# pangenome/povu

Hardware: AMD Instinct MI355X
Metric: edges/sec decomposed (flubble+PVST) (higher is better)
Workload: dtype u32

## Files before the change

include/povu_hip.h:

```cpp
#ifndef POVU_HIP_H
#define POVU_HIP_H

#include <stddef.h>
#include <stdint.h>

#ifdef __cplusplus
extern "C" {
#endif

#define POVU_HIP_NIL 0xFFFFFFFFu
#define POVU_SIDE_L 0
#define POVU_SIDE_R 1
#define POVU_TIP_NONE 0
#define POVU_TIP_L 1
#define POVU_TIP_R 2

typedef struct povu_hip_ctx povu_hip_ctx;
typedef struct povu_hip_forest povu_hip_forest;

int povu_hip_device_count(void);

povu_hip_ctx *povu_hip_create(int device, char *err, size_t errlen);
void povu_hip_destroy(povu_hip_ctx *ctx);
int povu_hip_release_workspace(povu_hip_ctx *ctx);
// ... 320 lines not shown
char *povu_hip_pvst_format(uint32_t n_pvst, const uint32_t *a_id, const uint32_t *z_id, const uint8_t *a_or,
			   const uint8_t *z_or, const uint32_t *parent, size_t *len);
char *povu_hip_pvst_format_fam(uint32_t n_pvst, const uint32_t *a_id, const uint32_t *z_id, const uint8_t *a_or,
			       const uint8_t *z_or, const uint32_t *parent, const uint8_t *fam, size_t *len);
void povu_hip_buffer_free(void *p);

typedef struct {
	uint32_t n;
	char *type;
	uint32_t *file_id;
	uint32_t *a_id, *z_id;
	uint8_t *a_or, *z_or;
	uint8_t *route;
	uint32_t *parent;
	uint32_t *height;
} povu_pvst_doc;
povu_pvst_doc *povu_pvst_parse(const char *text, size_t len, char *err, size_t errlen);

int povu_hip_gfa_write(const char *path, uint32_t n_vtx, const uint32_t *vid, uint32_t n_links, const uint32_t *v1,
		       const uint8_t *s1, const uint32_t *v2, const uint8_t *s2, char *err, size_t errlen);
void povu_pvst_doc_free(povu_pvst_doc *doc);

typedef struct {
	povu_hip_call_refs refs;
	uint32_t n_paths;
	const uint32_t *slot_of_path;
	const char *const *sample;
	const int64_t *slot_hap;
} povu_hip_call_names;
povu_hip_call_names *povu_hip_call_names_make(uint32_t n_paths, const char *const *path_name, uint32_t n_prefixes,
					      const char *const *prefix, char *err, size_t errlen);
void povu_hip_call_names_free(povu_hip_call_names *n);
int povu_hip_sites_add_tree(povu_hip_sites *s, uint32_t tree, uint32_t n, const uint32_t *id1, const uint32_t *id2,
			    const uint8_t *or1, const uint8_t *or2, const uint32_t *parent, const uint8_t *family);
povu_hip_sites *povu_hip_sites_of_docs(const povu_pvst_doc *const *docs, uint32_t n);
povu_hip_sites *povu_hip_forest_sites(const povu_hip_forest *f);
void povu_hip_sites_free(povu_hip_sites *s);
char *povu_hip_calls_vcf(const povu_hip_calls *c, const povu_hip_sites *sites, const povu_hip_call_names *names,
			 const char *const *path_name, const char *date, const char *only_prefix, uint32_t threads, size_t *len);
char *povu_hip_calls_vcf_profile(const povu_hip_calls *c, const povu_hip_sites *sites, const povu_hip_call_names *names,
				 const char *const *path_name, const char *date, const char *only_prefix, uint32_t threads, uint32_t profile,
				 size_t *len);
char *povu_hip_calls_vcf_rest(const povu_hip_calls *c, const povu_hip_sites *sites, const povu_hip_call_names *names,
			      const char *const *path_name, const char *date, const char *const *prefix, uint32_t n_prefixes, uint32_t threads,
			      uint32_t profile, size_t *len);

#define POVU_HIP_V_FOUND_FWD 0u
#define POVU_HIP_V_FOUND_REV 1u
#define POVU_HIP_V_ABSENT 2u
#define POVU_HIP_V_NO_AT 3u
#define POVU_HIP_V_BAD_STEP 4u
#define POVU_HIP_V_NO_SLOT 5u
#define POVU_HIP_V_MISSPELLED 6u
#define POVU_HIP_V_N_STATUS 6u
#define POVU_HIP_V_SPELL_NONE 0u
#define POVU_HIP_V_SPELL_WHOLE 1u
#define POVU_HIP_V_SPELL_ANCHORED 2u
#define POVU_HIP_V_SPELL_MISSPELLED 3u
#define POVU_HIP_V_FORWARD_ONLY 1u
#define POVU_HIP_V_SPELLING 2u
#define POVU_HIP_V_FORCE_TIER2 4u
typedef struct {
	uint64_t n_samples, n_records, n_alleles, n_steps, n_text_bytes, n_tasks, n_id_bytes;
	const char *const *sample;
	const uint64_t *rec_line;
	const uint64_t *rec_pos;
	const uint64_t *rec_id_off;
	const char *ids;
	const uint64_t *allele_off;
	const uint64_t *task_off;
	const uint64_t *step_off;
	const uint64_t *text_off;
	const uint8_t *allele_walk;
	const uint32_t *step_id;
	const uint8_t *step_or;
	const char *text;
	const uint32_t *task_record, *task_allele, *task_col, *task_phase;
} povu_hip_vcf_doc;
povu_hip_vcf_doc *povu_hip_vcf_parse(const char *text, size_t len, uint32_t threads, char *err, size_t errlen);
void povu_hip_vcf_doc_free(povu_hip_vcf_doc *d);
povu_hip_call_names *povu_hip_vcf_names_make(uint32_t n_paths, const char *const *path_name, char *err, size_t errlen);
int povu_hip_vcf_columns(const povu_hip_vcf_doc *doc, const povu_hip_call_names *names, uint32_t *col_first, uint32_t *col_slots);
typedef struct {
	uint32_t flags;
} povu_hip_vcf_opts;
typedef struct {
	uint64_t n_records, n_tasks, n_alleles;
	const uint8_t *task_status;
	const uint8_t *allele_spell;
	const uint8_t *rec_invalid;
	const uint8_t *rec_reason;
	const uint32_t *rec_allele, *rec_task;
	uint64_t n_status[POVU_HIP_V_N_STATUS];
	uint64_t n_invalid, n_misspelled;
	uint64_t n_tier2;
	double device_ms;
} povu_hip_vcf_report;
povu_hip_vcf_report *povu_hip_vcf_check(povu_hip_ctx *ctx, const povu_hip_vcf_doc *doc, const povu_hip_call_names *names,
					const povu_hip_vcf_opts *opts, char *err, size_t errlen);
void povu_hip_vcf_report_free(povu_hip_vcf_report *r);
char *povu_hip_vcf_report_text(const povu_hip_vcf_report *r, const povu_hip_vcf_doc *doc, const povu_hip_call_names *names,
			       size_t *report_len, char **summary, size_t *summary_len);

typedef struct {
	char name[48];
	double ms;
	uint32_t launches;
} povu_hip_stage_time;
int povu_hip_last_stage_times(const povu_hip_ctx *ctx, povu_hip_stage_time *out, int max);
uint32_t povu_hip_last_seq_redo(const povu_hip_ctx *ctx);
int povu_hip_last_black_only_classes(const povu_hip_ctx *ctx);
int povu_hip_last_narrow_counts(const povu_hip_ctx *ctx);
uint64_t povu_hip_wide_repeats(const povu_hip_ctx *ctx);
int povu_hip_last_laminar_check_ran(const povu_hip_ctx *ctx);
int povu_hip_last_crossings(povu_hip_ctx *ctx, uint32_t out[2]);
uint64_t povu_hip_last_links_processed(const povu_hip_ctx *ctx);

int povu_hip_debug_components(povu_hip_ctx *ctx, uint32_t *comp_of, uint32_t *local_idx);
int povu_hip_debug_tree(povu_hip_ctx *ctx, uint32_t comp, uint32_t *n_tree, uint32_t *gid, uint8_t *typ,
			uint32_t *par, uint32_t *cls);
int povu_hip_debug_edge_ids(povu_hip_ctx *ctx, uint32_t comp, uint32_t *n_tree, uint32_t *tree_edge_id);
int povu_hip_debug_walk_words(povu_hip_ctx *ctx, uint32_t out[3]);
int povu_hip_debug_stack(povu_hip_ctx *ctx, uint32_t comp, uint32_t *n, uint32_t *tree_vtx, uint32_t *cls,
			 uint32_t *next_seen);

#define POVU_HIP_SCAN_SUM 0
#define POVU_HIP_SCAN_MAX 1
#define POVU_HIP_SCAN_U64 2
#define POVU_HIP_SCAN_U8 3
#define POVU_HIP_SCAN_DIFF 4
#define POVU_HIP_SCAN_XOR_PAIR 5
#define POVU_HIP_SCAN_XOR_U128 6
#define POVU_HIP_SCAN_DIFF_U8 7
#define POVU_HIP_SCAN_MIXED_PAIR 8
#define POVU_HIP_SCAN_DIFF_U8_U8 9
#define POVU_HIP_SCAN_IN_PLACE 0x100
#define POVU_HIP_SCAN_N_DEV 0x200
int povu_hip_debug_scan(povu_hip_ctx *ctx, int op, const uint32_t *in, uint32_t *out, size_t n, const uint32_t *in2,
			uint32_t *out2, size_t n2);
int povu_hip_debug_sort(povu_hip_ctx *ctx, const uint32_t *keys, const uint32_t *vals, size_t n, unsigned bits,
			uint32_t *keys_out, uint32_t *vals_out);
int povu_hip_debug_compact(povu_hip_ctx *ctx, const uint8_t *flags, size_t n, uint32_t *out, uint32_t *count);
int povu_hip_debug_totals(povu_hip_ctx *ctx, const uint32_t *a, const uint32_t *b, size_t n, uint64_t tot[2]);
#define POVU_HIP_SEG_MIN 0
#define POVU_HIP_SEG_FIRST_LESS 1
#define POVU_HIP_SEG_LAST_LESS 2
int povu_hip_debug_segtree(povu_hip_ctx *ctx, const uint32_t *val, size_t n, const uint32_t *queries, size_t nq, uint32_t *out,
			   uint32_t *tree, uint32_t *P);
int povu_hip_debug_bitrank(povu_hip_ctx *ctx, const uint8_t *flags, size_t n, const uint32_t *pos, size_t nq, uint32_t *rank,
			   uint32_t *test, uint32_t *records);
int povu_hip_debug_append(povu_hip_ctx *ctx, const uint8_t *flags, size_t n, uint32_t *list, uint32_t *count);
int povu_hip_debug_list_rank(povu_hip_ctx *ctx, uint32_t n, const uint32_t *next, const uint8_t *w, const uint32_t *heads,
			     uint32_t nh, int mode, uint32_t bits, uint32_t *ra, uint32_t *rb);
double povu_hip_debug_scan_time(povu_hip_ctx *ctx, size_t n, int reps, int op);

uint64_t povu_hip_workspace_estimate(uint32_t n_vtx, uint32_t n_links, uint32_t n_components);
int povu_hip_workspace_breakdown(uint32_t n_vtx, uint32_t n_links, uint32_t n_components, uint64_t out[7]);
int povu_hip_prewarm(povu_hip_ctx *ctx, uint32_t n_vtx, uint32_t n_links, char *err, size_t errlen);
uint64_t povu_hip_leaf_workspace_estimate(uint32_t n_vtx, uint32_t n_components);

const char *povu_hip_version(void);

#ifdef __cplusplus
}
#endif
#endif
```

povu_amd/csrc/hip/context.hpp:

```cpp
#pragma once
#include "../../../include/povu_hip.h"

#include "forest_wire.hpp"
#include "graph_kernels.hpp"
#include "leaf_kernels.hpp"
#include "par_kernels.hpp"
#include "seq_kernels.hpp"
#include "sub_kernels.hpp"
#include "tree_kernels.hpp"

#include <map>
#include <memory>
#include <mutex>
#include <numeric>
#include <string>

using namespace povu_hip;

struct PinnedPool {
	struct Block {
		void *p;
		size_t cap;
		int seg;
	};
// ... 53 lines not shown
			return;
		if (from && from->shared_tag.empty()) {
			pool = from;
			p = static_cast<T *>(pool->get(m * sizeof(T), cap_bytes, &seg));
		} else {
			p = static_cast<T *>(malloc(m * sizeof(T)));
			if (!p)
				throw std::bad_alloc();
		}
		n = m;
	}
	void assign(size_t m, T v)
	{
		resize(m);
		std::fill(p, p + m, v);
	}
	void assign(const T *a, const T *b)
	{
		resize((size_t)(b - a));
		if (n)
			memcpy(p, a, n * sizeof(T));
	}
	T *data() { return p; }
	const T *data() const { return p; }
	T *begin() { return p; }
	const T *begin() const { return p; }
	size_t size() const { return n; }
	bool empty() const { return n == 0; }
	T &operator[](size_t i) { return p[i]; }
	const T &operator[](size_t i) const { return p[i]; }
};

struct povu_hip_forest {
	uint32_t total_components = 0;
	hipEvent_t ev0 = nullptr, ev1 = nullptr;
	bool pending = false;
	double pass_ms = -1.0;
	std::vector<hipEvent_t> more_events;
	std::once_flag ready_once;
	void wait_arrays()
	{
		if (pending) {
			if (ev1)
				(void)hipEventSynchronize(ev1);
			for (hipEvent_t e : more_events)
				(void)hipEventSynchronize(e);
			pending = false;
		}
	}
	void ready()
	{
		std::call_once(ready_once, [this] {
			wait_arrays();
			float ms = 0;
			if (ev0 && ev1 && pass_ms < 0 && hipEventElapsedTime(&ms, ev0, ev1) == hipSuccess)
				pass_ms = ms;
		});
	}
	std::shared_ptr<PinnedPool> pool;
	size_t meta_reserve = 0;
	static size_t meta_bytes(size_t n_trees) { return 64 + 32 * n_trees; }
	using Arrays = forest_wire::PvstArrays;
	static size_t block_bytes_for(size_t total) { return Arrays::layout(nullptr, total) + 64; }
	struct Block : Arrays {
		void *p = nullptr;
		size_t cap = 0, bytes = 0, total = 0;
		int seg = -1;
		std::shared_ptr<PinnedPool> pool;
		PinnedVec<uint32_t> sub_ai, sub_zi;
		PinnedVec<uint8_t> sub_fam;
		std::shared_ptr<SubForest> subx;
	};
	std::vector<Block> blocks;
	bool labels = false;
	Block &alloc(size_t total, void *q = nullptr, size_t cap = 0)
	{
		Block b;
		b.total = total, b.p = q, b.cap = cap;
		if (!q) {
			b.pool = pool;
			b.p = pool->get(block_bytes_for(total) + meta_bytes(meta_reserve), b.cap, &b.seg);
		}
		b.bytes = Arrays::layout(b.p, total, &b);
		blocks.push_back(std::move(b));
		return blocks.back();
	}
	void release_blocks()
	{
		for (auto &b : blocks)
			if (b.p && b.pool)
				b.pool->put(b.p, b.cap, b.seg);
		blocks.clear();
	}
	~povu_hip_forest()
	{
		std::call_once(ready_once, [this] { wait_arrays(); });
		if (ev0)
			(void)hipEventDestroy(ev0);
		if (ev1)
			(void)hipEventDestroy(ev1);
		for (hipEvent_t e : more_events)
			(void)hipEventDestroy(e);
		release_blocks();
		if (xblk && pool)
			pool->put(xblk, xblk_cap, xblk_seg);
	}
	struct Tree : forest_wire::TreeRecord {
		int blk = 0;
	};
	std::vector<Tree> trees;
	std::vector<uint64_t> hairpins;
	void *xblk = nullptr;
	size_t xblk_cap = 0;
	int xblk_seg = -1;
	const void *walk_ctx = nullptr;
	uint64_t walk_gen = 0;
};

struct PassPlan {
	uint32_t rank = 0, world = 1;
	bool hairpins = false, all_seq = false, seq_tree = false, par_tree = true, leaf_sub = false, all_sub = false;
	bool sorted_adj = false, force_redo = false, redo_odd = false;
	bool big_class_dfs = false, sparse_splitters = false, all_vertex_classes = false, check_laminar = false;
	bool timed = true, overlap_tail = false, heaviest_first = false;
};

struct LastPass {
	bool valid = false;
	PassPlan plan;
	uint32_t C = 0, seq_redo = 0;
	bool mixed = false, redo_pvst_only = false, stack_export_pending = false;
	bool narrow_counts = false;
	int narrow_forms = 0;
};

struct povu_hip_ctx {
	int device = 0;
	hipStream_t stream = nullptr;
	SideStream side;
	ResidentGraph g;
	SubArenas ws_sub;
	Arena ws, ws_b, ws2, ws_seq, ws_leaf, ws_walk, upload_tmp;
	HostScratch host;
	std::shared_ptr<PinnedPool> pool = std::make_shared<PinnedPool>();
	StageTimer timer;
	std::vector<povu_hip_stage_time> last_times;
	uint64_t last_links = 0;
	uint64_t wide_repeats = 0;
	CompState cs{};
	SeqWs sw{};
	ParWs pw{};
	TreeWs tw{};
	LastPass last;
	std::vector<uint32_t> shard_comp_ids;
	uint32_t shard_total_components = 0;
	Arena shard_buf;
	Arena graph_arena;
	hipEvent_t tail_done = nullptr;
	SideStream walk_side;
	bool tail_pending = false;
	void wait_tail()
	{
		if (tail_pending) {
			(void)hipEventSynchronize(tail_done);
			tail_pending = false;
		}
	}
	void quiesce()
	{
		if (tail_pending) {
			(void)hipStreamSynchronize(stream);
			wait_tail();
		}
	}
	Arena wk_ws, wk_out;
	Arena paths_buf;
	uint32_t *path_steps = nullptr;
	uint64_t *path_off = nullptr;
	uint32_t n_paths = 0;
	uint64_t n_path_steps = 0, paths_gen = 0;
	bool paths_valid = false;
	Arena tr_ws, tr_task, tr_trav, tr_steps;
	Arena seq_buf, cl_ws, cl_slot, cl_rec, cl_spell, cl_bytes;
	Arena iv_ws, iv_heads, iv_rows;
	Arena nm_ws;
	Arena pr_ws, pr_slab, pr_rows;
	Arena mg_ws, mg_rows;
	Arena ns_idx, ns_cls, ns_ws, ns_rec;
	Arena or_ws, or_view, or_inv, or_host, or_rows;
	Arena vc_ws, vc_hit;
	uint64_t *seq_off = nullptr;
	char *seq = nullptr;
	uint64_t seq_gen = 0;
	bool seq_valid = false;
	Arena part_arena;
	uint64_t xfer_h2d = 0, xfer_d2h = 0, xfer_peer_out = 0, xfer_peer_in = 0;
	struct Mapped {
		void *p;
		size_t bytes;
	};
	std::map<std::string, Mapped> attached;
};

struct XferScope {
	povu_hip_ctx *ctx;
	XferTally at;
	explicit XferScope(povu_hip_ctx *c) : ctx(c), at(xfer_tally()) {}
	~XferScope()
	{
		if (!ctx)
			return;
		const XferTally now = xfer_tally();
		ctx->xfer_h2d += now.h2d - at.h2d;
		ctx->xfer_d2h += now.d2h - at.d2h;
	}
};


void adopt_forest(povu_hip_forest &out, povu_hip_forest &m);

static inline void lpt_assign(const uint64_t *weights, uint32_t n, uint32_t world, uint32_t *order, uint32_t *owner)
{
	std::iota(order, order + n, 0u);
	std::stable_sort(order, order + n, [&](uint32_t a, uint32_t b) { return weights[a] > weights[b]; });
	std::vector<uint64_t> load(world, 0);
	for (uint32_t k = 0; k < n; k++) {
		const uint32_t c = order[k];
		uint32_t best = 0;
		for (uint32_t r = 1; r < world; r++)
			if (load[r] < load[best])
				best = r;
		owner[c] = best;
		load[best] += weights[c] + 1;
	}
}

void alloc_resident_graph(Arena &arena, ResidentGraph &g, uint32_t n_vtx, uint32_t n_links, bool tips_given);
void free_resident_graph(ResidentGraph &g);
void check_graph_size(uint32_t n_vtx, uint32_t n_links);
void set_err(char *err, size_t errlen, const std::string &msg);

struct Sizes {
	size_t V, E, Cmax, T, B, nS, slots;
	void set_components(size_t C) { Cmax = C, T = 2 * V + C, B = E + V + 2 * T; }
};
struct RowBNeeds {
	bool identity;
	bool sort_free;
	bool self_loops;
};
size_t rowb_carve_label(Arena *ar, const Sizes &z, CompState &cs);
size_t rowb_carve_reindex(Arena *ar, const Sizes &z, size_t C, const RowBNeeds &need, CompState &cs);
size_t carve_workspace(Arena *ar, int part, const Sizes &z, CompState &cs, SeqWs &sw, bool hairpins);
```

povu_amd/csrc/hip/debug_hooks.hip:

```cpp
#include "context.hpp"
#include "segtree.hpp"

#include <algorithm>
#include <numeric>

using namespace povu_hip;

namespace
{
constexpr size_t DBG_GUARD = 256;
constexpr int DBG_GUARD_BYTE = 0xC5, DBG_POISON_BYTE = 0xA7;
constexpr int DBG_RC_GUARD = 5;
struct DbgOut {
	size_t bytes = 0;
	int fill = DBG_GUARD_BYTE;
	bool on = true;
	char *base = nullptr;
	size_t span = 0;
	template <class T>
	T *data() const { return reinterpret_cast<T *>(base + DBG_GUARD); }
	void declare(Spans &take, hipStream_t s)
	{
		if (!on)
			return;
// ... 246 lines not shown
	for (uint32_t j = 0; j < 4 && t0 + j < n; j++)
		f |= (flags[t0 + j] ? 1u : 0u) << j;
	const uint32_t w0 = (BIDX * blockDim.x + (threadIdx.x & ~63u)) / 16u;
	bitrank_store_wave(rec + w0, f, w0 + (threadIdx.x & 63u) <= n / 64u);
}
__global__ void __launch_bounds__(256) k_dbg_bitrank_query(uint32_t n, const uint4 *__restrict__ rec, uint32_t nq, const uint32_t *__restrict__ x,
							   uint32_t *__restrict__ rank, uint32_t *__restrict__ test)
{
	for (uint32_t i = blockIdx.x * blockDim.x + threadIdx.x; i < nq; i += gridDim.x * blockDim.x) {
		const uint32_t p = x[i];
		rank[i] = bitrank(rec, p);
		if (p < n)
			test[i] = bitrank_test(rec, p) ? 1u : 0u;
	}
}
__global__ void __launch_bounds__(LIST_TPB) k_dbg_append(uint32_t n, const uint8_t *__restrict__ flags, uint32_t *__restrict__ list,
							  uint32_t *__restrict__ n_list)
{
	const uint32_t B0 = BIDX * LIST_SPAN;
	unsigned long long fw = 0;
#pragma unroll
	for (uint32_t it = 0; it < LIST_ITER; it++) {
		const uint32_t p0 = B0 + it * (LIST_TPB * 4u) + threadIdx.x * 4u;
		uint32_t f = 0;
		for (uint32_t j = 0; j < 4 && p0 + j < n; j++)
			f |= (flags[p0 + j] ? 1u : 0u) << j;
		fw |= (unsigned long long)f << (4 * it);
	}
	append_in_order(fw, B0, list, n_list);
}
constexpr size_t DBG_LOOKUP_MAX_N = (size_t(1) << 32) - (size_t(1) << 16);
unsigned dbg_query_blocks(size_t nq) { return (unsigned)std::min<size_t>(std::max<size_t>((nq + 255) / 256, 1), 4096); }
}

extern "C" int povu_hip_debug_segtree(povu_hip_ctx *ctx, const uint32_t *val, size_t n, const uint32_t *queries, size_t nq, uint32_t *out,
				      uint32_t *tree, uint32_t *P)
{
	if (!ctx || n > DBG_LOOKUP_MAX_N || nq >= (size_t(1) << 32) || (n && !val) || (nq && (!queries || !out)))
		return 1;
	for (size_t i = 0; i < nq; i++)
		if (queries[4 * i] > DBG_SEG_LAST || queries[4 * i + 2] > n)
			return 1;
	try {
		HIP_CHECK(hipSetDevice(ctx->device));
		hipStream_t s = ctx->stream;
		const size_t padded = (n + SEG_BLK - 1) / SEG_BLK * SEG_BLK, tw = SegTree::tree_words(n);
		Arena ar;
		DbgOut ot{tw * 4, DBG_POISON_BYTE}, oq{nq * 4};
		DbgScratch vals{(padded + SEG_BLK) * 4};
		DbgIn<uint32_t> dq{queries, 4 * nq};
		dbg_carve(ar, s, ot, oq, vals, dq);
		uint32_t *dv = static_cast<uint32_t *>(vals.p);
		if (n)
			HIP_CHECK(copy_async(dv, val, n * 4, hipMemcpyHostToDevice, s));
		if (padded > n)
			HIP_CHECK(hipMemsetAsync(dv + n, 0, (padded - n) * 4, s));
		SegTree st;
		st.tree = ot.data<uint32_t>();
		seg_build(st, dv, n, s);
		if (nq)
			KLAUNCH(k_dbg_seg_query, dim3(dbg_query_blocks(nq)), dim3(256), 0, s, st, (uint32_t)nq, reinterpret_cast<const uint4 *>(dq.dev), oq.data<uint32_t>());
		std::vector<uint32_t> ht(tw);
		HIP_CHECK(copy_async(ht.data(), ot.data<char>(), tw * 4, hipMemcpyDeviceToHost, s));
		if (nq)
			HIP_CHECK(copy_async(out, oq.data<char>(), nq * 4, hipMemcpyDeviceToHost, s));
		HIP_CHECK(hipStreamSynchronize(s));
		if (P)
			*P = st.P;
		if (tree)
			std::copy(ht.begin(), ht.begin() + 2 * (size_t)st.P, tree);
		if (!dbg_guards_intact(ot, s) || !dbg_guards_intact(oq, s))
			return DBG_RC_GUARD;
		const unsigned char *hb = reinterpret_cast<const unsigned char *>(ht.data());
		for (size_t i = 2 * (size_t)st.P * 4; i < tw * 4; i++)
			if (hb[i] != (unsigned char)DBG_POISON_BYTE)
				return DBG_RC_GUARD;
		return 0;
	} catch (const std::exception &) {
		return 2;
	}
}

extern "C" int povu_hip_debug_bitrank(povu_hip_ctx *ctx, const uint8_t *flags, size_t n, const uint32_t *pos, size_t nq, uint32_t *rank,
				      uint32_t *test, uint32_t *records)
{
	if (!ctx || n > DBG_LOOKUP_MAX_N || nq >= (size_t(1) << 32) || (n && !flags) || (nq && (!pos || !rank || !test)))
		return 1;
	for (size_t i = 0; i < nq; i++)
		if (pos[i] > n)
			return 1;
	try {
		HIP_CHECK(hipSetDevice(ctx->device));
		hipStream_t s = ctx->stream;
		const size_t n_rec = n / 64 + 1, tb = scan_tmp_bytes(n_rec + 1);
		Arena ar;
		DbgOut orec{(n_rec + 1) * 16, DBG_POISON_BYTE}, ocnt{(n_rec + 1) * 4, DBG_POISON_BYTE}, ork{nq * 4}, ots{nq * 4};
		DbgScratch tmp{tb};
		DbgIn<uint8_t> df{flags, n};
		DbgIn<uint32_t> dp{pos, nq};
		dbg_carve(ar, s, orec, ocnt, ork, ots, tmp, df, dp);
		uint4 *rec = orec.data<uint4>();
		const size_t waves = n / 256 + 1;
		KLAUNCH(k_dbg_bitrank_flags, dim3((unsigned)((waves * 64 + 255) / 256)), dim3(256), 0, s, (uint32_t)n, df.dev, rec);
		bitrank_build(rec, n_rec, ocnt.data<uint32_t>(), tmp.p, tb, s);
		if (nq) {
			KLAUNCH(k_dbg_bitrank_query, dim3(dbg_query_blocks(nq)), dim3(256), 0, s, (uint32_t)n, rec, (uint32_t)nq, dp.dev, ork.data<uint32_t>(),
				ots.data<uint32_t>());
			HIP_CHECK(copy_async(rank, ork.data<char>(), nq * 4, hipMemcpyDeviceToHost, s));
			HIP_CHECK(copy_async(test, ots.data<char>(), nq * 4, hipMemcpyDeviceToHost, s));
		}
		if (records)
			HIP_CHECK(copy_async(records, orec.data<char>(), (n_rec + 1) * 16, hipMemcpyDeviceToHost, s));
		HIP_CHECK(hipStreamSynchronize(s));
		return dbg_guards_intact(orec, s) && dbg_guards_intact(ocnt, s) && dbg_guards_intact(ork, s) && dbg_guards_intact(ots, s) ? 0 : DBG_RC_GUARD;
	} catch (const std::exception &) {
		return 2;
	}
}

extern "C" int povu_hip_debug_append(povu_hip_ctx *ctx, const uint8_t *flags, size_t n, uint32_t *list, uint32_t *count)
{
	if (!ctx || !count || n > DBG_LOOKUP_MAX_N || (n && (!flags || !list)))
		return 1;
	try {
		HIP_CHECK(hipSetDevice(ctx->device));
		hipStream_t s = ctx->stream;
		Arena ar;
		DbgOut ol{n * 4}, oc{4};
		DbgIn<uint8_t> df{flags, n};
		dbg_carve(ar, s, ol, oc, df);
		HIP_CHECK(hipMemsetAsync(oc.data<char>(), 0, 4, s));
		if (n)
			KLAUNCH(k_dbg_append, dim3((unsigned)((n + LIST_SPAN - 1) / LIST_SPAN)), dim3(LIST_TPB), 0, s, (uint32_t)n, df.dev, ol.data<uint32_t>(),
				oc.data<uint32_t>());
		if (n)
			HIP_CHECK(copy_async(list, ol.data<char>(), n * 4, hipMemcpyDeviceToHost, s));
		HIP_CHECK(copy_async(count, oc.data<char>(), 4, hipMemcpyDeviceToHost, s));
		HIP_CHECK(hipStreamSynchronize(s));
		if (!dbg_guards_intact(ol, s) || !dbg_guards_intact(oc, s))
			return DBG_RC_GUARD;
		return dbg_all_guard(list, std::min<size_t>(*count, n) * 4, n * 4) ? 0 : DBG_RC_GUARD;
	} catch (const std::exception &) {
		return 2;
	}
}

extern "C" int povu_hip_debug_list_rank(povu_hip_ctx *ctx, uint32_t n, const uint32_t *next, const uint8_t *w, const uint32_t *heads,
					uint32_t nh, int mode, uint32_t bits, uint32_t *ra, uint32_t *rb)
{
	if (!ctx || !next || !w || (nh && !heads) || !ra || (mode != 0 && !rb) || mode < 0 || mode > 1)
		return 1;
	try {
		HIP_CHECK(hipSetDevice(ctx->device));
		debug_list_rank(n, next, w, heads, nh, mode, bits, ra, rb, ctx->stream);
		return 0;
	} catch (const std::exception &) {
		return 2;
	}
}

extern "C" double povu_hip_debug_scan_time(povu_hip_ctx *ctx, size_t n, int reps, int op)
{
	if (!ctx || !n || reps <= 0)
		return -1.0;
	try {
		HIP_CHECK(hipSetDevice(ctx->device));
		hipStream_t s = ctx->stream;
		Arena ar;
		const size_t tb = scan_tmp_bytes(n);
		uint32_t *di = nullptr, *dout = nullptr;
		void *tmp = nullptr;
		carve(ar, [&](Spans &take) {
			take(n + 16, di, dout);
			take(tb, tmp);
		});
		HIP_CHECK(hipMemsetAsync(di, 1, n * 4, s));
		hipEvent_t e0, e1;
		HIP_CHECK(hipEventCreate(&e0));
		HIP_CHECK(hipEventCreate(&e1));
		for (int w = 0; w < 2; w++)
			op ? scan_exclusive_max_u32(di, dout, n, tmp, tb, s) : scan_exclusive_u32(di, dout, n, tmp, tb, s);
		HIP_CHECK(hipEventRecord(e0, s));
		for (int r = 0; r < reps; r++)
			op ? scan_exclusive_max_u32(di, dout, n, tmp, tb, s) : scan_exclusive_u32(di, dout, n, tmp, tb, s);
		HIP_CHECK(hipEventRecord(e1, s));
		HIP_CHECK(hipEventSynchronize(e1));
		float ms = 0;
		HIP_CHECK(hipEventElapsedTime(&ms, e0, e1));
		(void)hipEventDestroy(e0);
		(void)hipEventDestroy(e1);
		return (double)ms / reps;
	} catch (const std::exception &) {
		return -2.0;
	}
}

extern "C" int povu_hip_debug_components(povu_hip_ctx *ctx, uint32_t *comp_of, uint32_t *local_idx)
{
	if (!ctx || !ctx->last.valid)
		return 1;
	ctx->quiesce();
	try {
		HIP_CHECK(hipSetDevice(ctx->device));
		const uint32_t V = ctx->g.V, C = ctx->last.C;
		std::vector<uint32_t> pos(V), voff(C + 1);
		HIP_CHECK(hipMemcpy(comp_of, ctx->cs.comp_of, (size_t)V * 4, hipMemcpyDeviceToHost));
		if (ctx->cs.lean_identity)
			std::iota(pos.begin(), pos.end(), 0u);
		else
			HIP_CHECK(hipMemcpy(pos.data(), ctx->cs.pos, (size_t)V * 4, hipMemcpyDeviceToHost));
		HIP_CHECK(hipMemcpy(voff.data(), ctx->cs.voff, (size_t)(C + 1) * 4, hipMemcpyDeviceToHost));
		for (uint32_t v = 0; v < V; v++)
			local_idx[v] = pos[v] - voff[comp_of[v]];
		return 0;
	} catch (const std::exception &) {
		return 2;
	}
}

extern "C" int povu_hip_debug_tree(povu_hip_ctx *ctx, uint32_t comp, uint32_t *n_tree, uint32_t *gid, uint8_t *typ,
				   uint32_t *par, uint32_t *cls)
{
	if (!ctx || !ctx->last.valid || comp >= ctx->last.C || !n_tree)
		return 1;
	if (cls && ctx->last.mixed)
		return 4;
	ctx->quiesce();
	try {
		HIP_CHECK(hipSetDevice(ctx->device));
		uint32_t voff = 0, N = 0;
		HIP_CHECK(hipMemcpy(&voff, ctx->cs.voff + comp, 4, hipMemcpyDeviceToHost));
		HIP_CHECK(hipMemcpy(&N, ctx->sw.c_ntree + comp, 4, hipMemcpyDeviceToHost));
		*n_tree = N;
		const size_t tb = 2 * (size_t)voff + comp;
		if (gid)
			HIP_CHECK(hipMemcpy(gid, ctx->sw.t_gid + tb, (size_t)N * 4, hipMemcpyDeviceToHost));
		if (par)
			HIP_CHECK(hipMemcpy(par, ctx->sw.t_par + tb, (size_t)N * 4, hipMemcpyDeviceToHost));
		const bool par_cls = !ctx->last.plan.all_seq && (ctx->last.seq_redo == 0 || ctx->last.redo_pvst_only);
		if (cls && par_cls) {
			classes_to_tree_space(ctx->pw, ctx->stream);
			HIP_CHECK(hipStreamSynchronize(ctx->stream));
		}
		if (cls)
			HIP_CHECK(hipMemcpy(cls, (par_cls ? ctx->pw.gcls : ctx->sw.t_cls) + tb, (size_t)N * 4, hipMemcpyDeviceToHost));
		if (typ)
			HIP_CHECK(hipMemcpy(typ, ctx->sw.t_flags + tb, N, hipMemcpyDeviceToHost));
		return 0;
	} catch (const std::exception &) {
		return 2;
	}
}

extern "C" int povu_hip_debug_edge_ids(povu_hip_ctx *ctx, uint32_t comp, uint32_t *n_tree, uint32_t *tree_edge_id)
{
	if (!ctx || !ctx->last.valid || comp >= ctx->last.C || !n_tree)
		return 1;
	if (!ctx->last.plan.par_tree)
		return 3;
	if (ctx->last.mixed)
		return 4;
	uint32_t *dw = nullptr;
	ctx->quiesce();
	try {
		HIP_CHECK(hipSetDevice(ctx->device));
		uint32_t voff = 0, N = 0;
		HIP_CHECK(hipMemcpy(&voff, ctx->cs.voff + comp, 4, hipMemcpyDeviceToHost));
		HIP_CHECK(hipMemcpy(&N, ctx->sw.c_ntree + comp, 4, hipMemcpyDeviceToHost));
		*n_tree = N;
		if (!tree_edge_id || N == 0)
			return 0;
		const size_t T = 2 * (size_t)ctx->sw.V + ctx->last.C, tb = 2 * (size_t)voff + comp;
		HIP_CHECK(hipMalloc(reinterpret_cast<void **>(&dw), 2 * T * 4));
		HIP_CHECK(hipMemsetAsync(dw, 0, 2 * T * 4, ctx->stream));
		edge_id_weights(ctx->cs, ctx->sw, ctx->tw, dw, dw + T, ctx->stream);
		std::vector<uint32_t> w(N), tail(N), size(N);
		HIP_CHECK(copy_async(w.data(), dw + tb, (size_t)N * 4, hipMemcpyDeviceToHost, ctx->stream));
		HIP_CHECK(copy_async(tail.data(), dw + T + tb, (size_t)N * 4, hipMemcpyDeviceToHost, ctx->stream));
		HIP_CHECK(copy_async(size.data(), ctx->sw.t_size + tb, (size_t)N * 4, hipMemcpyDeviceToHost, ctx->stream));
		HIP_CHECK(hipStreamSynchronize(ctx->stream));
		HIP_CHECK(hipFree(dw));
		dw = nullptr;
		std::vector<uint32_t> closed((size_t)N + 1, 0);
		for (uint32_t t = 0; t < N; t++)
			closed[std::min<size_t>((size_t)t + size[t], N)] += tail[t];
		uint32_t before = 0;
		tree_edge_id[0] = POVU_NIL;
		for (uint32_t t = 0; t < N; t++) {
			before += w[t] + closed[t];
			if (t > 0)
				tree_edge_id[t] = t - 1 + before;
		}
		return 0;
	} catch (const std::exception &) {
		if (dw)
			(void)hipFree(dw);
		return 2;
	}
}

extern "C" int povu_hip_debug_walk_words(povu_hip_ctx *ctx, uint32_t out[3])
{
	if (!ctx || !ctx->last.valid || !out)
		return 1;
	if (!ctx->last.plan.par_tree)
		return 3;
	if (ctx->last.mixed)
		return 4;
	ctx->quiesce();
	try {
		HIP_CHECK(hipSetDevice(ctx->device));
// ... 40 lines not shown
```

povu_amd/csrc/hip/tree_kernels.hip:

```cpp
#include "tree_kernels.hpp"

#include <cstdlib>

#include <algorithm>
#include <type_traits>
#include <vector>

namespace povu_hip
{

#ifndef NIL
#define NIL POVU_NIL
#endif

static unsigned rank_bucket_bits(size_t n)
{
	if (const char *ev = getenv("POVU_HIP_RANK_BITS"))
		return (unsigned)std::min(6, std::max(2, atoi(ev)));
	(void)n;
	return 3u;
}
static constexpr uint32_t PK_END = 0x1FFFFFFFu, PK_STOP = 0x80000000u;
static constexpr uint32_t P0_END = 0x3FFFFFFFu, P0_W = 0x40000000u, P0_HEAD = 0x80000000u;
static constexpr uint32_t FT_NONE = 0x7FFFFFFFu, FT_HASH = 0x80000000u;
// ... 96 lines not shown
				h = hx(h, link_hash(le));
				continue;
			}
			if (first == NIL)
				first = at;
			const uint32_t w = ws[q], sb = o01[q].x;
			const uint32_t wl = (w & 1u) ? o01[q].y : sb, wh = (w & 1u) ? se[q] : o01[q].y;
			uint32_t nxt;
			if (se[q] - sb <= 8) {
				const uint32_t n = se[q] - sb, tl = wl - sb, th = wh - sb;
				uint4 c = make_uint4(0u, 0u, 0u, 0u);
				if (n > 4)
					c = load4_unaligned(lle + sb + 4);
				const uint32_t r[8] = {a[q].x, a[q].y, a[q].z, a[q].w, c.x, c.y, c.z, c.w};
				uint32_t tk = 0, first_tree = NIL, after = NIL;
#pragma unroll
				for (uint32_t k = 0; k < 8; k++)
					if (k >= tl && k < th && (r[k] & LLE_ID) == le)
						tk = k;
#pragma unroll
				for (uint32_t k = 0; k < 8; k++)
					if (k < n && (r[k] & LLE_TREE)) {
						if (first_tree == NIL)
							first_tree = k;
						if (k > tk && after == NIL)
							after = k;
					}
				nxt = sb + (after != NIL ? after : (first_tree < tk ? first_tree : tk));
			} else {
				const uint32_t t = wl + find_link_slot(loff, lle, w, le) - 1;
				nxt = t;
				for (uint32_t jj = t + 1; jj < se[q] && nxt == t; jj++)
					if (lle[jj] & LLE_TREE)
						nxt = jj;
				for (uint32_t jj = sb; jj < t && nxt == t; jj++)
					if (lle[jj] & LLE_TREE)
						nxt = jj;
			}
			pk[at] = rank_pack(nxt, 1u, b);
		}
	}
	const bool nz = !hzero(h);
	if (nz)
		hside[S] = h;
	ft[S] = (first == NIL ? FT_NONE : first) | (nz ? FT_HASH : 0u);
}
__device__ __forceinline__ uint32_t comp_root_side(const unsigned long long *start_key, const uint32_t *voff, uint32_t c)
{
	unsigned long long k = start_key[c];
	return k == ~0ull ? 2 * voff[c] : (uint32_t)(k & 0xFFFFFFFFu);
}
__global__ void k_tour_ends(uint32_t C, const uint32_t *__restrict__ voff, const unsigned long long *__restrict__ start_key,
			    const uint32_t *__restrict__ loff, const uint32_t *__restrict__ ladj, const uint32_t *__restrict__ lle,
			    uint32_t *__restrict__ pk, uint32_t *__restrict__ heads)
{
	uint32_t c = BIDX * blockDim.x + threadIdx.x;
	if (c >= C)
		return;
	const uint32_t r = comp_root_side(start_key, voff, c), sb = loff[r & ~1u], se = loff[(r & ~1u) + 2], mid = loff[r];
	uint32_t a_first = NIL, a_last = NIL;
	for (uint32_t j = mid; j < se; j++)
		if (lle[j] & LLE_TREE) {
			if (a_first == NIL)
				a_first = j;
			a_last = j;
		}
	for (uint32_t j = sb; j < mid; j++)
		if (lle[j] & LLE_TREE) {
			if (a_first == NIL)
				a_first = j;
			a_last = j;
		}
	heads[c] = a_first;
	if (a_first == NIL)
		return;
	pk[arc_twin(loff, ladj, lle, a_last)] = P0_END;
	atomicOr(&pk[a_first], P0_HEAD);
}
template <int HOPS>
__global__ void k_wyllie(uint32_t n, const uint32_t *__restrict__ nxt_in, const uint32_t *__restrict__ a_in,
			 const uint32_t *__restrict__ b_in, uint32_t *__restrict__ nxt_out, uint32_t *__restrict__ a_out,
			 uint32_t *__restrict__ b_out, const uint32_t *__restrict__ n_dev)
{
	uint32_t i = BIDX * blockDim.x + threadIdx.x;
	if (i >= n || (n_dev && i >= *n_dev))
		return;
	uint32_t nx = nxt_in[i], a = a_in[i], b = b_in ? b_in[i] : 0;
#pragma unroll
	for (int hop = 0; hop < HOPS; hop++) {
		if (nx == NIL)
			break;
		a += a_in[nx];
		if (b_in)
			b += b_in[nx];
		nx = nxt_in[nx];
	}
	nxt_out[i] = nx;
	a_out[i] = a;
	if (b_out)
		b_out[i] = b;
}
static int list_rank(uint32_t n, unsigned bits, uint32_t *nxtA, uint32_t *nxtB, uint32_t *aA, uint32_t *aB, uint32_t *bA,
		     uint32_t *bB, hipStream_t s, const uint32_t *n_dev = nullptr)
{
	int cur = 0;
	const bool small = n < (1u << 21);
	const unsigned launches = small ? (bits + 2) / 3 : (bits + 1) / 2;
	for (unsigned r = 0; r < launches; r++) {
		uint32_t *ni = cur ? nxtB : nxtA, *no = cur ? nxtA : nxtB, *ai = cur ? aB : aA, *ao = cur ? aA : aB;
		uint32_t *bi = cur ? bB : bA, *bo = cur ? bA : bB;
		if (small)
			LAUNCH(k_wyllie<7>, n, s, n, ni, ai, bi, no, ao, bo, n_dev);
		else
			LAUNCH(k_wyllie<3>, n, s, n, ni, ai, bi, no, ao, bo, n_dev);
		cur ^= 1;
	}
	return cur;
}

static constexpr uint32_t RANK_TOP = 8192;
struct RankLevelArgs {
	uint32_t n;
	uint32_t m;
	uint32_t hbase;
	uint32_t M;
};
template <bool L0>
__device__ __forceinline__ uint32_t rank_lane_start(uint32_t id, const RankLevelArgs &A, unsigned b, const uint32_t *__restrict__ pk0,
						    const uint32_t *__restrict__ heads)
{
	if (id < A.m) {
		const uint32_t x = bucket_splitter(id, b);
		if (x >= A.n)
			return NIL;
		if (L0)
			return (pk0[x] & P0_HEAD) ? NIL : x;
		return x >= A.hbase ? NIL : x;
	}
	return L0 ? heads[id - A.m] : A.hbase + (id - A.m);
}
template <bool EVT3>
__device__ __forceinline__ void rank_l0_weights(uint32_t x, uint32_t p, uint32_t &wa, uint32_t &wb)
{
	if (EVT3) {
		const uint32_t t = x % 3u;
		wa = t == 0 ? 2u : 0u;
		wb = t == 0 ? 2u : ((t == 1 && (p & P0_W)) ? 0u - 2u : 0u - 1u);
	} else {
		wa = (p & P0_W) ? 1u : 0u;
		wb = wa ? 1u : 0xFFFFFFFFu;
	}
}
static constexpr uint32_t REC_MAX = 0xFFFFu;
template <bool L0, bool TWO, bool EVT3 = false>
__global__ void k_rank_up(RankLevelArgs A, unsigned b, const uint32_t *__restrict__ nx_in, const uint32_t *__restrict__ a_in,
			  const uint32_t *__restrict__ b_in, const uint32_t *__restrict__ heads, uint32_t *__restrict__ nx_out,
			  uint32_t *__restrict__ a_out, uint32_t *__restrict__ b_out, uint2 *__restrict__ rec, uint32_t *__restrict__ ovf)
{
	const uint32_t id = BIDX * blockDim.x + threadIdx.x;
	if (id >= A.M)
		return;
	uint32_t x = rank_lane_start<L0>(id, A, b, nx_in, heads);
	uint32_t sa = 0, sb = 0, out = PK_END | PK_STOP;
	bool big = false;
	if (x != NIL) {
		uint32_t p;
		bool stop;
		do {
			p = nx_in[x];
			if (L0) {
				uint32_t wa, wb;
				rank_l0_weights<EVT3>(x, p, wa, wb);
				if (TWO) {
					big |= sa > REC_MAX || sa - sb > REC_MAX;
					rec[x] = make_uint2(id, sa | ((sa - sb) << 16));
				} else {
					rec[x] = make_uint2(id, sa);
				}
				sa += wa;
				if (TWO)
					sb += wb;
				x = p & P0_END;
				stop = rank_l0_stop(x, b);
			} else {
				sa += a_in[x];
				if (TWO)
					sb += b_in[x];
				x = p & PK_END;
				stop = (p & PK_STOP) != 0;
			}
		} while (!stop);
		if (x != (L0 ? P0_END : PK_END)) {
			const uint32_t q = x >> b;
			out = q | (is_splitter(q, b) ? PK_STOP : 0u);
		}
	}
	nx_out[id] = out;
	a_out[id] = sa;
	if (TWO)
		b_out[id] = sb;
	if (L0 && TWO && big)
		*ovf = 1u;
}
template <bool EVT3>
__global__ void k_rank_l0_fallback(RankLevelArgs A, unsigned b, const uint32_t *__restrict__ pk, const uint32_t *__restrict__ heads,
				   const uint32_t *__restrict__ ra, const uint32_t *__restrict__ rb, uint2 *__restrict__ rec,
				   const uint32_t *__restrict__ ovf)
{
	if (!*ovf)
		return;
	for (uint32_t id = BIDX * blockDim.x + threadIdx.x; id < A.M; id += gridDim.x * blockDim.x) {
		uint32_t x = rank_lane_start<true>(id, A, b, pk, heads);
		if (x == NIL)
			continue;
		uint32_t sa = ra[id], sb = rb[id];
		do {
			const uint32_t p = pk[x];
			uint32_t wa, wb;
			rank_l0_weights<EVT3>(x, p, wa, wb);
			rec[x] = make_uint2(sa, sb);
			sa -= wa;
			sb -= wb;
			x = p & P0_END;
		} while (!rank_l0_stop(x, b));
	}
}
template <bool TWO>
__global__ void k_rank_down(RankLevelArgs A, unsigned b, const uint32_t *__restrict__ nx_in, uint32_t *a_io, uint32_t *b_io,
			    const uint32_t *__restrict__ ra, const uint32_t *__restrict__ rb)
{
	const uint32_t id = BIDX * blockDim.x + threadIdx.x;
	if (id >= A.M)
		return;
	uint32_t x = rank_lane_start<false>(id, A, b, nx_in, nullptr);
	if (x == NIL)
		return;
	uint32_t sa = ra[id], sb = TWO ? rb[id] : 0, p;
	do {
		p = nx_in[x];
		const uint32_t wa = a_io[x];
		a_io[x] = sa;
		sa -= wa;
		if (TWO) {
			const uint32_t wb = b_io[x];
			b_io[x] = sb;
			sb -= wb;
		}
		x = p & PK_END;
	} while (!(p & PK_STOP));
}
template <bool TWO>
__global__ void __launch_bounds__(1024) k_rank_top(uint32_t n, const uint32_t *__restrict__ nx_in, uint32_t *a_io, uint32_t *b_io)
{
	__shared__ uint32_t nx[RANK_TOP], sa[RANK_TOP], sb[TWO ? RANK_TOP : 1];
	for (uint32_t i = threadIdx.x; i < n; i += blockDim.x) {
		const uint32_t p = nx_in[i] & PK_END;
		nx[i] = p == PK_END ? NIL : p;
		sa[i] = a_io[i];
		if (TWO)
			sb[i] = b_io[i];
	}
	__syncthreads();
	constexpr int PER = RANK_TOP / 1024;
	for (uint32_t span = 1; span < n; span <<= 1) {
		uint32_t tn[PER], ta[PER], tb[PER];
#pragma unroll
		for (int k = 0; k < PER; k++) {
			const uint32_t i = threadIdx.x + k * 1024;
			tn[k] = NIL, ta[k] = 0, tb[k] = 0;
			if (i < n && nx[i] != NIL) {
				const uint32_t j = nx[i];
				tn[k] = nx[j];
				ta[k] = sa[j];
				if (TWO)
					tb[k] = sb[j];
			}
		}
		__syncthreads();
#pragma unroll
		for (int k = 0; k < PER; k++) {
			const uint32_t i = threadIdx.x + k * 1024;
			if (i < n && nx[i] != NIL) {
				nx[i] = tn[k];
				sa[i] += ta[k];
				if (TWO)
					sb[i] += tb[k];
			}
		}
		__syncthreads();
	}
	for (uint32_t i = threadIdx.x; i < n; i += blockDim.x) {
		a_io[i] = sa[i];
		if (TWO)
			b_io[i] = sb[i];
	}
}
__global__ void k_rank_unpack_next(uint32_t n, const uint32_t *__restrict__ nx_in, uint32_t *__restrict__ out)
{
	uint32_t i = BIDX * blockDim.x + threadIdx.x;
	if (i < n) {
		const uint32_t p = nx_in[i] & PK_END;
		out[i] = p == PK_END ? NIL : p;
	}
}

struct RankBufs {
	uint32_t *pk;
	uint32_t *heads;
	uint32_t *nx, *wa, *wb;
	uint32_t *tA, *tB, *tC;
};
static constexpr int RANK_MAX_LEVELS = 12;
static size_t rank_pool_words(size_t n, size_t nh) { return n / 2 + 4 * nh + 64; }

struct L0Ranks {
	const uint32_t *ra, *rb, *fin;
	uint32_t M;
};
__device__ __forceinline__ uint32_t l0_at(const L0Ranks &R, uint2 rec, bool want = true) { return want && rec.x < R.M ? rec.x : 0u; }
__device__ __forceinline__ uint32_t rank_l0(const L0Ranks &R, uint2 rec, uint32_t ra) { return (rec.x < R.M ? ra : 0u) - rec.y; }
__device__ __forceinline__ uint32_t rank_l0_a(const L0Ranks &R, uint2 rec, bool fin, uint32_t ra)
{
	return fin ? rec.x : (rec.x < R.M ? ra : 0u) - (rec.y & REC_MAX);
}
__device__ __forceinline__ uint2 rank_l0_pair(const L0Ranks &R, uint2 rec, bool fin, uint32_t ra, uint32_t rb)
{
	const bool in = rec.x < R.M;
	const uint32_t pa = rec.y & REC_MAX;
	return fin ? rec : make_uint2((in ? ra : 0u) - pa, (in ? rb : 0u) - pa + (rec.y >> 16));
}
__device__ __forceinline__ uint32_t rank_l0(const L0Ranks &R, uint2 rec) { return rank_l0(R, rec, R.ra[l0_at(R, rec)]); }
__device__ __forceinline__ uint2 rank_l0_pair(const L0Ranks &R, uint2 rec, bool fin)
{
	const uint32_t i = l0_at(R, rec, !fin);
	return rank_l0_pair(R, rec, fin, R.ra[i], R.rb[i]);
}

template <bool TWO, bool EVT3 = false>
static L0Ranks list_rank_splitters(uint32_t n, unsigned b, uint2 *rec, uint32_t *ovf, uint32_t nh, RankBufs &rb, hipStream_t s)
{
	if (n >= P0_END)
		throw HipError("list ranking: more than 2^30 elements (graph too large for the packed walk)");
	RankLevelArgs lv[RANK_MAX_LEVELS];
	uint32_t *nxp[RANK_MAX_LEVELS + 1], *wap[RANK_MAX_LEVELS + 1], *wbp[RANK_MAX_LEVELS + 1];
	int levels = 0;
	size_t used = 0;
	const size_t pool = rank_pool_words(n, nh);
	nxp[0] = rb.pk, wap[0] = wbp[0] = nullptr;
	uint32_t cur_n = n, hbase = 0;
	for (;;) {
		RankLevelArgs &A = lv[levels];
		A.n = cur_n;
		A.m = (cur_n + (1u << b) - 1) >> b;
		A.hbase = hbase;
		A.M = A.m + nh;
		if (used + A.M > pool)
			throw HipError("list ranking: level pool exhausted (internal sizing bug)");
		nxp[levels + 1] = rb.nx + used, wap[levels + 1] = rb.wa + used, wbp[levels + 1] = rb.wb + used;
		used += A.M;
		levels++;
		hbase = A.m;
		const uint32_t next_n = A.M;
		if (next_n <= RANK_TOP || next_n > cur_n / 2 || levels == RANK_MAX_LEVELS) {
			cur_n = next_n;
			break;
		}
		cur_n = next_n;
	}
	if (TWO)
		HIP_CHECK(hipMemsetAsync(ovf, 0, 4, s));
	for (int L = 0; L < levels; L++) {
		const RankLevelArgs &A = lv[L];
		if (L == 0)
			LAUNCH((k_rank_up<true, TWO, EVT3>), A.M, s, A, b, nxp[0], nullptr, nullptr, rb.heads, nxp[1], wap[1], wbp[1], rec, ovf);
		else
			LAUNCH((k_rank_up<false, TWO>), A.M, s, A, b, nxp[L], wap[L], wbp[L], nullptr, nxp[L + 1], wap[L + 1], wbp[L + 1],
			       nullptr, nullptr);
	}
	const uint32_t nt = cur_n;
	if (nt <= RANK_TOP) {
		KLAUNCH((k_rank_top<TWO>), dim3(1), dim3(1024), 0, s, nt, nxp[levels], wap[levels], wbp[levels]);
	} else {
		LAUNCH(k_rank_unpack_next, nt, s, nt, nxp[levels], rb.tA);
		HIP_CHECK(copy_async(rb.tB, wap[levels], (size_t)nt * 4, hipMemcpyDeviceToDevice, s));
		if (TWO)
			HIP_CHECK(copy_async(rb.tC, wbp[levels], (size_t)nt * 4, hipMemcpyDeviceToDevice, s));
		uint32_t *nA = rb.tA, *nB = nxp[levels], *aA = rb.tB, *aB = wap[levels], *bA = rb.tC, *bB = wbp[levels];
		const int side = list_rank(nt, bits_for(nt) + 1, nA, nB, aA, aB, TWO ? bA : nullptr, TWO ? bB : nullptr, s);
		if (side == 0) {
			HIP_CHECK(copy_async(wap[levels], aA, (size_t)nt * 4, hipMemcpyDeviceToDevice, s));
			if (TWO)
				HIP_CHECK(copy_async(wbp[levels], bA, (size_t)nt * 4, hipMemcpyDeviceToDevice, s));
		}
	}
	for (int L = levels - 1; L >= 1; L--) {
		const RankLevelArgs &A = lv[L];
		LAUNCH((k_rank_down<TWO>), A.M, s, A, b, nxp[L], wap[L], wbp[L], wap[L + 1], wbp[L + 1]);
	}
	if (TWO)
		KLAUNCH((k_rank_l0_fallback<EVT3>), dim3(std::min(nblk(lv[0].M), 2048u)), dim3(TPB), 0, s, lv[0], b, rb.pk, rb.heads, wap[1],
			wbp[1], rec, ovf);
	return L0Ranks{wap[1], TWO ? wbp[1] : nullptr, TWO ? ovf : nullptr, lv[0].M};
}

template <bool TWO>
__global__ void k_rank_resolve(uint32_t n, const uint2 *__restrict__ rec, L0Ranks R, uint32_t *__restrict__ ra, uint32_t *__restrict__ rb)
{
	const uint32_t x = BIDX * blockDim.x + threadIdx.x;
	if (x >= n)
		return;
	if (TWO) {
		const uint2 r = rank_l0_pair(R, rec[x], *R.fin != 0);
		ra[x] = r.x;
		rb[x] = r.y;
	} else {
		ra[x] = rank_l0(R, rec[x]);
	}
}
void debug_list_rank(uint32_t n, const uint32_t *next, const uint8_t *w, const uint32_t *heads, uint32_t nh, int mode,
		     unsigned bits, uint32_t *ra, uint32_t *rb, hipStream_t s)
{
	if (n == 0 || n >= P0_END)
		throw HipError("debug_list_rank: n must be in [1, 2^30)");
	const unsigned b = bits ? std::min(6u, std::max(2u, bits)) : rank_bucket_bits(n);
	std::vector<uint32_t> pk(n);
	for (uint32_t x = 0; x < n; x++) {
		if (next[x] != NIL && next[x] >= n)
			throw HipError("debug_list_rank: successor out of range");
		pk[x] = (next[x] == NIL ? P0_END : next[x]) | (w[x] ? P0_W : 0u);
	}
	for (uint32_t h = 0; h < nh; h++)
		if (heads[h] != NIL) {
			if (heads[h] >= n)
				throw HipError("debug_list_rank: head out of range");
			pk[heads[h]] |= P0_HEAD;
		}
	const size_t pool = rank_pool_words(n, nh);
	Arena ar;
	ar.reserve(Arena::padded(n + 16, 4) * 3 + Arena::padded(n + 16, 8) + Arena::padded(nh + 1, 4) + 6 * Arena::padded(pool, 4) + 8192, false);
	RankBufs rbf{};
	rbf.pk = ar.take<uint32_t>(n + 16);
	rbf.heads = ar.take<uint32_t>(nh + 1);
	for (uint32_t **q : {&rbf.nx, &rbf.wa, &rbf.wb, &rbf.tA, &rbf.tB, &rbf.tC})
		*q = ar.take<uint32_t>(pool);
	uint32_t *da = ar.take<uint32_t>(n + 16), *db = ar.take<uint32_t>(n + 16), *ovf = ar.take<uint32_t>(4);
	uint2 *rec = ar.take<uint2>(n + 16);
	HIP_CHECK(copy_async(rbf.pk, pk.data(), (size_t)n * 4, hipMemcpyHostToDevice, s));
	if (nh)
		HIP_CHECK(copy_async(rbf.heads, heads, (size_t)nh * 4, hipMemcpyHostToDevice, s));
	if (mode == 0) {
		const L0Ranks R = list_rank_splitters<false>(n, b, rec, nullptr, nh, rbf, s);
		LAUNCH(k_rank_resolve<false>, n, s, n, rec, R, da, nullptr);
	} else {
		const L0Ranks R = list_rank_splitters<true, true>(n, b, rec, ovf, nh, rbf, s);
		LAUNCH(k_rank_resolve<true>, n, s, n, rec, R, da, db);
	}
	HIP_CHECK(copy_async(ra, da, (size_t)n * 4, hipMemcpyDeviceToHost, s));
	if (mode != 0)
		HIP_CHECK(copy_async(rb, db, (size_t)n * 4, hipMemcpyDeviceToHost, s));
	HIP_CHECK(hipStreamSynchronize(s));
}

static constexpr uint32_t T0_RBIT = 0x80000000u;
static constexpr uint32_t BS_POS = 0x3FFFFFFFu, BS_NOARC = 0x80000000u, BS_HASH_L = 0x40000000u, BS_HASH_R = 0x80000000u;
__global__ void k_t0_parents(uint32_t V, const uint2 *__restrict__ trec, L0Ranks R, const uint32_t *__restrict__ ckey,
			     const uint32_t *__restrict__ voff, const uint32_t *__restrict__ loff, const uint32_t *__restrict__ ladj,
			     const uint32_t *__restrict__ lle,
			     const uint32_t *__restrict__ ft, const uint32_t *__restrict__ heads,
			     uint4 *__restrict__ t0seg, uint2 *__restrict__ fstr, uint4 *__restrict__ xrec, uint32_t C,
			     const unsigned long long *__restrict__ start_key, uint32_t *__restrict__ err, uint8_t *__restrict__ multi)
{
	uint32_t g = BIDX * blockDim.x + threadIdx.x;
	if (g < V)
		*reinterpret_cast<uint16_t *>(multi + 2 * g) = 0;
	if (g < C) {
		const uint32_t r = comp_root_side(start_key, voff, g), L = 2 * (voff[g + 1] - voff[g] - 1);
		t0seg[r >> 1] = make_uint4(NIL, (r & 1u) ? T0_RBIT : 0u, 0u, L ? L - 1 : 0u);
		const uint32_t h = heads[g];
		if (h == NIL ? L != 0 : rank_l0(R, trec[h]) != L - 1)
			atomicExch(err, 1u);
	}
	if (g >= V)
		return;
	const uint32_t sb = loff[2 * g], sm = loff[2 * g + 1], se = loff[2 * g + 2];
	const uint2 f2 = *reinterpret_cast<const uint2 *>(ft + 2 * g);
	uint32_t at_e = NIL, dmin = 0xFFFFFFFFu, dmax = 0u;
	uint32_t a_l = NIL, a_r = NIL, d_l = 0u, d_r = 0u;
	for (uint32_t at0 = sb; at0 < se; at0 += 4) {
		const uint32_t *r32 = reinterpret_cast<const uint32_t *>(trec + at0);
		const uint4 lw4 = load4_unaligned(lle + at0), r01 = load4_unaligned(r32), r23 = load4_unaligned(r32 + 4);
		const uint32_t lws[4] = {lw4.x, lw4.y, lw4.z, lw4.w};
		const uint2 rs[4] = {make_uint2(r01.x, r01.y), make_uint2(r01.z, r01.w), make_uint2(r23.x, r23.y), make_uint2(r23.z, r23.w)};
		bool tree[4];
		uint32_t ds[4];
#pragma unroll
		for (uint32_t q = 0; q < 4; q++) {
			tree[q] = at0 + q < se && (lws[q] & LLE_TREE);
			ds[q] = R.ra[l0_at(R, rs[q], tree[q])];
		}
		landed(ds[0], ds[1], ds[2], ds[3]);
#pragma unroll
		for (uint32_t q = 0; q < 4; q++)
			ds[q] = rank_l0(R, rs[q], ds[q]);
#pragma unroll
		for (uint32_t q = 0; q < 4; q++) {
			if (!tree[q])
				continue;
			if (ds[q] < dmin) {
				dmin = ds[q];
				at_e = at0 + q;
			}
			dmax = max(dmax, ds[q]);
			if (at0 + q < sm) {
				if (a_l == NIL)
					a_l = at0 + q, d_l = ds[q];
			} else if (a_r == NIL) {
				a_r = at0 + q, d_r = ds[q];
			}
		}
	}
	const uint32_t hbits = ((f2.x & FT_HASH) ? BS_HASH_L : 0u) | ((f2.y & FT_HASH) ? BS_HASH_R : 0u);
	if (at_e == NIL) {
		fstr[g] = make_uint2(BS_NOARC, hbits);
		return;
	}
	const uint32_t c = ckey[g], root = comp_root_side(start_key, voff, c);
	const uint32_t L = 2 * (voff[c + 1] - voff[c] - 1), abase = 2 * (voff[c] - c);
	if ((root >> 1) == g) {
		const bool far_r = !(root & 1u);
		const uint32_t a1 = far_r ? a_r : a_l, d1 = far_r ? d_r : d_l;
		fstr[g] = a1 == NIL ? make_uint2(BS_NOARC, hbits) : make_uint2((abase + (L - 1 - d1)) & BS_POS, ((abase + L) & BS_POS) | hbits);
		return;
	}
	const uint32_t p_in = abase + (L - 2 - dmax), p_out = abase + (L - 1 - dmin);
	t0seg[g] = make_uint4(ladj[at_e], (lle[at_e] & LLE_ID) | (at_e >= sm ? T0_RBIT : 0u), p_in, p_out);
	{
		const bool ent_r = at_e >= sm;
		const uint32_t a1 = ent_r ? a_l : a_r, d1 = ent_r ? d_l : d_r, a3 = ent_r ? a_r : a_l, d3 = ent_r ? d_r : d_l;
		const uint32_t end = a3 != at_e ? abase + (L - 1 - d3) : p_out;
		fstr[g] = a1 == NIL ? make_uint2(BS_NOARC, hbits) : make_uint2((abase + (L - 1 - d1)) & BS_POS, (end & BS_POS) | hbits);
	}
	if ((f2.x | f2.y) & FT_HASH)
		atomicOr(reinterpret_cast<unsigned long long *>(&xrec[p_in >> 6]), 1ull << (p_in & 63u));
}
__global__ void k_tour_values(uint32_t V, const uint4 *__restrict__ t0seg, const uint32_t *__restrict__ ft,
			      const ulonglong2 *__restrict__ hside, const uint4 *__restrict__ xrec, ulonglong2 *__restrict__ xval)
{
	uint32_t g = BIDX * blockDim.x + threadIdx.x;
	if (g >= V)
		return;
	const uint2 f2 = *reinterpret_cast<const uint2 *>(ft + 2 * g);
	if (!((f2.x | f2.y) & FT_HASH))
		return;
	const uint4 r = t0seg[g];
	if (r.x == NIL)
		return;
	const ulonglong2 z = make_ulonglong2(0ull, 0ull);
	xval[bitrank(xrec, r.z)] = hx((f2.x & FT_HASH) ? hside[2 * g] : z, (f2.y & FT_HASH) ? hside[2 * g + 1] : z);
}
static constexpr uint32_t PB_BRIDGE = 0x80000000u;
static constexpr uint32_t CLASS_BUDGET = 256;
static constexpr uint32_t CS_VISITED = 0x40000000u;
__global__ void k_bridges(uint32_t V, const uint4 *__restrict__ t0seg, const uint2 *__restrict__ fstr,
			  const ulonglong2 *__restrict__ xps, const uint4 *__restrict__ xrec,
			  const ulonglong2 *__restrict__ hside, const uint32_t *__restrict__ loff, const uint32_t *__restrict__ lle,
			  const uint32_t *__restrict__ ckey, const uint32_t *__restrict__ cproc,
			  uint8_t *multi, uint32_t *__restrict__ cstate, uint2 *__restrict__ dps)
{
	const uint32_t g = BIDX * blockDim.x + threadIdx.x;
	if (g >= V)
		return;
	auto stretch = [&](uint32_t p, uint32_t q) {
		const uint32_t rp = bitrank(xrec, p), rq = bitrank(xrec, q);
		return rp == rq ? make_ulonglong2(0ull, 0ull) : hx(xps[rp], xps[rq]);
	};
	const uint4 r = t0seg[g];
	const uint32_t Se = (2 * g) | (r.y >> 31), Sf = Se ^ 1u, c = ckey[g];
	const bool proc = cproc[c] != 0;
	uint32_t pvE;
	if (r.x == NIL) {
		pvE = NIL;
	} else if (hzero(stretch(r.z, r.w + 1))) {
		pvE = r.x | PB_BRIDGE;
	} else {
		pvE = r.x;
		multi[Se] = 1;
		multi[r.x] = 1;
	}
	const uint2 fs = fstr[g];
	ulonglong2 x = (fs.y & ((Sf & 1u) ? BS_HASH_R : BS_HASH_L)) ? hside[Sf] : make_ulonglong2(0ull, 0ull);
	if (!(fs.x & BS_NOARC))
		x = hx(x, stretch(fs.x & BS_POS, fs.y & BS_POS));
	uint32_t pvF;
	if (hzero(x)) {
		pvF = Se | PB_BRIDGE;
	} else {
		pvF = Se;
		multi[Sf] = 1;
		multi[Se] = 1;
	}
	const bool entryE = proc && (pvE & PB_BRIDGE), entryF = proc && (pvF & PB_BRIDGE);
	const uint32_t csE = proc ? (pvE | (entryE ? CS_VISITED : 0u)) : NIL, csF = proc ? (pvF | (entryF ? CS_VISITED : 0u)) : NIL;
	uint2 recE = make_uint2(NIL, 0u), recF = make_uint2(NIL, 0u);
	if (entryE && pvE != NIL) {
		const uint32_t p = pvE & ~PB_BRIDGE;
		recE.x = p;
		uint32_t le = r.y & ~T0_RBIT, lo = loff[p], hi = loff[p + 1];
		while (lo < hi) {
			const uint32_t mid = (lo + hi) >> 1;
			if ((lle[mid] & LLE_ID) < le)
				lo = mid + 1;
			else
				hi = mid;
		}
		recE.y = lo - loff[p] + 1;
	}
	if (entryF)
		recF.x = Se;
	const bool e_first = !(Se & 1u);
	*reinterpret_cast<uint2 *>(cstate + 2 * g) = e_first ? make_uint2(csE, csF) : make_uint2(csF, csE);
	*reinterpret_cast<uint4 *>(dps + 2 * g) = e_first ? make_uint4(recE.x, recE.y, recF.x, recF.y) : make_uint4(recF.x, recF.y, recE.x, recE.y);
}


static constexpr uint32_t EL_ITER = LIST_ITER, EL_SIDES = LIST_SPAN;
static_assert(TPB == (int)LIST_TPB, "append_in_order is written for workgroups of 256");
__global__ void __launch_bounds__(TPB) k_entry_list(uint32_t nS, const uint32_t *__restrict__ pbr ,
						     const uint8_t *__restrict__ multi, const uint32_t *__restrict__ ckey,
						     const uint32_t *__restrict__ cproc, uint32_t *__restrict__ entry_list,
						     uint32_t *__restrict__ n_entry)
{
	const uint32_t B0 = BIDX * EL_SIDES;
	unsigned long long fw = 0;
#pragma unroll
	for (uint32_t it = 0; it < EL_ITER; it++) {
		const uint32_t S0 = B0 + it * (TPB * 4u) + threadIdx.x * 4u;
		uint32_t f = 0;
		if (S0 + 4 <= nS) {
			const uint4 pb = *reinterpret_cast<const uint4 *>(pbr + S0);
			const uint32_t mu = *reinterpret_cast<const uint32_t *>(multi + S0);
			const uint2 ck = *reinterpret_cast<const uint2 *>(ckey + (S0 >> 1));
			const uint32_t c0 = cproc[ck.x] ? 1u : 0u, c1 = cproc[ck.y] ? 1u : 0u;
			f = (((mu & 0xFFu) && (pb.x & PB_BRIDGE)) ? c0 : 0u) | ((((mu & 0xFF00u) && (pb.y & PB_BRIDGE)) ? c0 : 0u) << 1) |
			    ((((mu & 0xFF0000u) && (pb.z & PB_BRIDGE)) ? c1 : 0u) << 2) | ((((mu & 0xFF000000u) && (pb.w & PB_BRIDGE)) ? c1 : 0u) << 3);
		} else {
			for (uint32_t S = S0; S < nS; S++)
				f |= ((multi[S] && (pbr[S] & PB_BRIDGE) && cproc[ckey[S >> 1]]) ? 1u : 0u) << (S - S0);
		}
		fw |= (unsigned long long)f << (4 * it);
	}
// ... 260 lines not shown
						base = NIL;
					}
					chunk_base[n_chunks] = base;
				}
				base = sgpr(base);
				if (base == NIL) {
					pool_ok = false;
					return;
				}
				n_chunks++;
			}
			__syncthreads();
			if (lane < 32)
				wstk[wstk_addr(ev + lane, chunk_base)] = ring[(ev + lane) & 63u];
			lds_lo = ev + 32;
		}
		if (lane == 0)
			ring[d & 63u] = make_uint2(side, jn);
		depth = d + 1;
	};
	auto set_parent = [&](uint32_t side, uint32_t par) {
		const uint32_t kk = side - win_lo;
		if (HOT && kk < W_WIN) {
			if (lane == 0)
				win_par[kk] = par | W_DIRTY;
			return true;
		}
		if (lane == 0)
			wpar[side] = par;
		return false;
	};
#define W_INLINE_CAND(rr, idx, out)                                                                                            \
	do {                                                                                                                    \
		uint32_t v__ = (rr).c0;                                                                                         \
		v__ = (idx) == 1 ? (rr).c1 : v__;                                                                               \
		v__ = (idx) == 2 ? (rr).c2 : v__;                                                                               \
		v__ = (idx) == 3 ? (rr).c3 : v__;                                                                               \
		v__ = (idx) == 4 ? (rr).c4 : v__;                                                                               \
		v__ = (idx) == 5 ? (rr).c5 : v__;                                                                               \
		(out) = (idx) < (rr).n ? v__ : NIL;                                                                             \
	} while (0)
	constexpr uint32_t W_TRIAL = 512;
	uint32_t n_gen = 0, n_hot = 0;
	if (HOT) {
		for (;;) {
			if (n_gen >= W_TRIAL && n_hot < n_gen)
				break;
			n_gen++;
#define W_HOT 1
#include "walk_step.inc"
#undef W_HOT
		}
	}
	for (;;) {
#define W_HOT 0
#include "walk_step.inc"
#undef W_HOT
	}
}
__global__ void k_walk_finish(uint32_t nS, const uint32_t *__restrict__ wpar, const uint32_t *__restrict__ pbr,
			      const uint32_t *__restrict__ loff, const uint32_t *__restrict__ ladj, uint2 *__restrict__ dps)
{
	uint32_t S = BIDX * blockDim.x + threadIdx.x;
	if (S >= nS)
		return;
	const uint32_t p = wpar[S];
	if (p == W_UNVIS || (pbr[S] & PB_BRIDGE))
		return;
	uint32_t slot = 0;
	if (S != (p ^ 1u)) {
		const uint32_t lo = loff[p], hi = loff[p + 1];
		for (uint32_t k = lo; k < hi; k++)
			if (ladj[k] == S) {
				slot = k - lo + 1;
				break;
			}
	}
	dps[S] = make_uint2(p, slot);
}

__device__ __forceinline__ uint32_t leave_event(uint32_t p, bool p_is_far) { return 3 * (p >> 1) + (p_is_far ? 1u : 2u); }
__global__ void k_events(uint32_t V, const uint2 *__restrict__ dps, const uint32_t *__restrict__ loff,
			 const uint32_t *__restrict__ ladj, const uint32_t *__restrict__ ckey, const uint32_t *__restrict__ cproc,
			 uint32_t *__restrict__ pk, uint32_t *__restrict__ heads, unsigned b, uint8_t *__restrict__ merged,
			 uint32_t *__restrict__ sdl)
{
	const uint32_t g = BIDX * blockDim.x + threadIdx.x;
	if (g >= V)
		return;
	sdl[g] = 0;
	if (g == 0)
		sdl[V] = sdl[V + 1] = 0;
	const uint32_t A = 3 * g;
	const uint4 d4 = *reinterpret_cast<const uint4 *>(dps + 2 * g);
	if (d4.x != 2 * g + 1 && d4.z != 2 * g) {
		pk[A] = pk[A + 1] = pk[A + 2] = P0_END;
		merged[g] = 1;
		return;
	}
	const uint32_t o = d4.x == 2 * g + 1 ? 2 * g : 2 * g + 1, e = o ^ 1u;
	const uint32_t p = (e & 1u) ? d4.z : d4.x, slot_e = (e & 1u) ? d4.w : d4.y;
	auto child_behind = [&](uint32_t par, uint32_t lo, uint32_t n, uint32_t from) {
		for (uint32_t k = from; k <= n; k += 4) {
			const uint4 x = load4_unaligned(ladj + lo + k - 1);
			const uint32_t rem = n + 1 - k;
			const uint2 r0 = dps[x.x];
			const uint2 r1 = rem > 1 ? dps[x.y] : make_uint2(NIL, 0u);
			const uint2 r2 = rem > 2 ? dps[x.z] : make_uint2(NIL, 0u);
			const uint2 r3 = rem > 3 ? dps[x.w] : make_uint2(NIL, 0u);
			if (r0.x == par && r0.y == k)
				return x.x;
			if (r1.x == par && r1.y == k + 1)
				return x.y;
			if (r2.x == par && r2.y == k + 2)
				return x.z;
			if (r3.x == par && r3.y == k + 3)
				return x.w;
		}
		return NIL;
	};
	const uint2 s01 = *reinterpret_cast<const uint2 *>(loff + 2 * g);
	const uint32_t s2 = loff[2 * g + 2];
	const uint32_t lo_o = (o & 1u) ? s01.y : s01.x, n_o = ((o & 1u) ? s2 : s01.y) - lo_o;
	const uint32_t lo_e = (e & 1u) ? s01.y : s01.x, n_e = ((e & 1u) ? s2 : s01.y) - lo_e;
	const uint32_t c_o = child_behind(o, lo_o, n_o, 1u);
	const uint32_t ns_o = child_behind(e, lo_e, n_e, 1u);
	uint32_t after_e = NIL;
	if (p != NIL) {
		const uint32_t lo_p = loff[p], n_p = loff[p + 1] - lo_p;
		const uint32_t ns_e = child_behind(p, lo_p, n_p, slot_e + 1);
		after_e = ns_e != NIL ? 3 * (ns_e >> 1) : leave_event(p, dps[p].x == (p ^ 1u));
	}
	uint32_t enter = rank_pack(c_o != NIL ? 3 * (c_o >> 1) : A + 1, 0u, b);
	if (p == NIL) {
		const uint32_t comp = ckey[g];
		if (cproc[comp]) {
			enter |= P0_HEAD;
			heads[comp] = A;
		}
	}
	pk[A] = enter;
	if (ns_o != NIL) {
		pk[A + 1] = rank_pack(3 * (ns_o >> 1), 0u, b);
		pk[A + 2] = rank_pack(after_e, 0u, b);
		merged[g] = 0;
	} else {
		pk[A + 1] = rank_pack(after_e, 1u, b);
		pk[A + 2] = P0_END;
		merged[g] = 1;
	}
}

template <typename OC, typename SC, typename IC>
__global__ void k_tree_emit(uint32_t nS, const uint2 *__restrict__ erec, L0Ranks R, const uint8_t *__restrict__ merged,
			    const uint2 *__restrict__ dps, const uint32_t *__restrict__ ckey,
			    const uint32_t *__restrict__ cproc, const uint32_t *__restrict__ voff,
			    const unsigned long long *__restrict__ start_key, const uint32_t *__restrict__ gid_s,
			    uint32_t *__restrict__ t_gid, uint8_t *__restrict__ t_flags, uint32_t *__restrict__ t_par,
			    uint32_t *__restrict__ t_size, uint32_t *__restrict__ t_depth, uint32_t *__restrict__ side_tidx,
			    uint32_t C, uint32_t *__restrict__ c_ntree, OC *__restrict__ ordcnt, uint32_t *__restrict__ hi0,
			    uint32_t *__restrict__ mpre, SC *__restrict__ srccnt, uint32_t *__restrict__ sdl,
			    IC *__restrict__ incnt)
{
	uint32_t S = BIDX * blockDim.x + threadIdx.x;
	if (S == 0) {
		const uint32_t T = 2 * (nS >> 1) + C;
		hi0[T] = NIL;
		srccnt[T] = srccnt[T + 1] = 0;
		incnt[T] = incnt[T + 1] = 0;
	}
	if (S < C) {
		const uint32_t Nr = 2 * (voff[S + 1] - voff[S]), tr = 2 * voff[S] + S;
		if (!cproc[S]) {
			c_ntree[S] = 0;
			t_size[tr + Nr] = 0;
			srccnt[tr + Nr] = 0;
			incnt[tr + Nr] = 0;
		} else {
			const uint32_t hr = start_key[S] != ~0ull ? 1u : 0u;
			c_ntree[S] = Nr + hr;
			if (hr) {
				t_gid[tr] = NIL;
				t_flags[tr] = 2 | TF_ROOT;
				t_par[tr] = NIL;
				t_size[tr] = Nr + 1;
				incnt[tr] = 0;
				if (t_depth)
					t_depth[tr] = 0;
				mpre[tr] = tr;
				ordcnt[tr] = 0;
				hi0[tr] = NIL;
			} else {
				t_size[tr + Nr] = 0;
				srccnt[tr + Nr] = 0;
				incnt[tr + Nr] = 0;
			}
		}
	}
	const uint32_t g = S;
	if (g >= (nS >> 1))
		return;
	const uint32_t c = ckey[g], v0 = voff[c];
	const uint32_t tb = 2 * v0 + c;
	if (!cproc[c]) {
		const uint32_t t = tb + 2 * (g - v0);
		store2_unaligned(t_size + t, 0u, 0u);
		zero2(srccnt + t);
		zero2(incnt + t);
		*reinterpret_cast<uint2 *>(side_tidx + 2 * g) = make_uint2(NIL, NIL);
		return;
	}
	const uint32_t Nh = 2 * (voff[c + 1] - v0), hd = start_key[c] != ~0ull ? 1u : 0u;
	const bool fin = *R.fin != 0;
	const uint4 r01 = load4_unaligned(reinterpret_cast<const uint32_t *>(erec + 3 * g));
	const uint2 r2 = erec[3 * g + 2];
	const bool two_leaves = !merged[g];
	const uint4 d4 = *reinterpret_cast<const uint4 *>(dps + 2 * g);
	const uint32_t o = d4.x == 2 * g + 1 ? 2 * g : 2 * g + 1, e = o ^ 1u;
	const uint32_t p = (e & 1u) ? d4.z : d4.x;
	const bool has_p = p != NIL;
	const uint32_t pp = has_p ? p : e;
	const uint2 r_p = erec[3 * (pp >> 1)], d_p = dps[pp];
	const uint2 r0 = make_uint2(r01.x, r01.y), r1 = make_uint2(r01.z, r01.w);
	const uint32_t i0 = l0_at(R, r0, !fin);
	uint32_t a0 = R.ra[i0], b0 = R.rb[i0], a1 = R.ra[l0_at(R, r1, !fin)], a2 = R.ra[l0_at(R, r2, !fin && two_leaves)], a_p = R.ra[l0_at(R, r_p, !fin && has_p)];
	landed(a0, b0, a1, a2, a_p);
	const uint2 ent = rank_l0_pair(R, r0, fin, a0, b0), lv_o = make_uint2(rank_l0_a(R, r1, fin, a1), 0u);
	const uint32_t lv_e2 = rank_l0_a(R, r2, fin, a2), ent_p = rank_l0_a(R, r_p, fin, a_p);
	const uint32_t pre_e = Nh - ent.x, depth_e = 0u - ent.y;
	const uint32_t lv_e = two_leaves ? lv_e2 : lv_o.x;
	const uint32_t size_o = ent.x - 1 - lv_o.x, size_e = ent.x - lv_e;
	uint32_t par_e;
	if (!has_p)
		par_e = hd ? 0u : NIL;
	else
		par_e = hd + (Nh - ent_p) + (d_p.x == (p ^ 1u) ? 1u : 0u);
	const uint32_t l = hd + pre_e, t = tb + l;
	const uint32_t gid = gid_s[g];
	store2_unaligned(t_gid + t, gid, gid);
	t_flags[t] = (uint8_t)((e & 1u) | (par_e == NIL ? TF_ROOT : 0u));
	t_flags[t + 1] = (uint8_t)((o & 1u) | TF_BLACK);
	store2_unaligned(t_par + t, par_e, l);
	store2_unaligned(t_size + t, size_e, size_o);
	zero2(incnt + t);
	if (t_depth)
		store2_unaligned(t_depth + t, depth_e + hd, depth_e + 1 + hd);
	store2_unaligned(mpre + t, tb + (depth_e + hd) + (Nh + hd) - l - size_e, tb + (depth_e + 1 + hd) + (Nh + hd) - (l + 1) - size_o);
	*reinterpret_cast<uint2 *>(side_tidx + 2 * g) = (e & 1u) ? make_uint2(t + 1, t) : make_uint2(t, t + 1);
	if (sdl) {
		const uint32_t gray = (size_e - 1 - size_o) / 2, black = (size_o + 1) / 2, gs = v0 + pre_e / 2;
		if (gray) {
			atomicAdd(&sdl[gs], gray);
			atomicAdd(&sdl[gs + black], 0u - gray - black);
			atomicAdd(&sdl[gs + size_e / 2], black);
		}
	}
}
#ifndef POVU_BE_ITER
#define POVU_BE_ITER 8
#endif
static constexpr uint32_t BE_ITER = POVU_BE_ITER, BE_SIDES = TPB * BE_ITER;
template <bool EMIT, typename IC>
__device__ __forceinline__ uint32_t side_back_edges(uint32_t S, uint32_t p, uint32_t at,
						    const uint32_t *__restrict__ loff, const uint32_t *__restrict__ ladj,
						    const uint2 *__restrict__ dps, const uint32_t *__restrict__ side_tidx,
						    const uint32_t *__restrict__ ckey, const uint32_t *__restrict__ voff,
						    const uint32_t *__restrict__ t_par, uint32_t *__restrict__ b_src,
						    uint32_t *__restrict__ b_tgt, uint32_t *__restrict__ b_ord,
						    const uint8_t *__restrict__ dupflag, IC *__restrict__ incnt, uint32_t &highest,
						    uint32_t *first2)
{
	uint32_t n = 0;
	const uint32_t c = ckey[S >> 1], root = 2 * voff[c] + c;
	const uint32_t lo = loff[S], hi = loff[S + 1];
	auto out = [&](uint32_t tgt) {
		if (EMIT) {
			b_src[at + n] = p;
			b_tgt[at + n] = tgt;
			b_ord[at + n] = n;
			if (sizeof(IC) == 4 || tgt != root)
				incnt_add(incnt, tgt);
		} else {
			highest = min(highest, tgt);
			if (n < 2)
				first2[n] = tgt;
		}
		n++;
	};
	if (lo == hi) {
		if (p == root || t_par[p] != 0)
			out(root);
		return n;
	}
	const uint32_t dp = dps[S].x;
	bool loop_seen = false;
	for (uint32_t k0 = lo; k0 < hi; k0 += 4) {
		const uint4 o4 = load4_unaligned(ladj + k0);
		const uint32_t rem = hi - k0;
		const uint32_t os[4] = {o4.x, o4.y, o4.z, o4.w};
		const uint32_t xs[4] = {side_tidx[o4.x], rem > 1 ? side_tidx[o4.y] : NIL, rem > 2 ? side_tidx[o4.z] : NIL,
					rem > 3 ? side_tidx[o4.w] : NIL};
#pragma unroll
		for (uint32_t q = 0; q < 4; q++) {
			if (q >= rem)
				break;
			const uint32_t k = k0 + q, o = os[q], x = xs[q];
			if (o == (S ^ 1)) {
				if (dp == o && !loop_seen)
					out(x);
				loop_seen = true;
				continue;
			}
			if (x > p || o == dp)
				continue;
			bool dup = false;
			if (dupflag) {
				dup = dupflag[k] != 0;
			} else {
				for (uint32_t j = lo; j < k; j++)
					if (ladj[j] == o) {
						dup = true;
						break;
					}
			}
			if (!dup)
				out(x);
		}
	}
	return n;
}
template <typename OC, typename IC>
__global__ void __launch_bounds__(TPB) k_back_edges(uint32_t nS, const uint32_t *__restrict__ loff, const uint32_t *__restrict__ ladj,
						     const uint2 *__restrict__ dps, const uint32_t *__restrict__ side_tidx,
						     const uint32_t *__restrict__ ckey, const uint32_t *__restrict__ voff,
						     const uint32_t *__restrict__ t_par, uint32_t *__restrict__ total_out,
						     uint32_t *__restrict__ b_src, uint32_t *__restrict__ b_tgt,
						     uint32_t *__restrict__ b_ord, const uint8_t *__restrict__ dupflag,
						     OC *__restrict__ ordcnt, uint32_t *__restrict__ hi0, IC *__restrict__ incnt,
						     uint32_t cap)
{
	const uint32_t S0 = BIDX * BE_SIDES + threadIdx.x;
	__shared__ uint32_t first2[BE_ITER][TPB][2];
	__shared__ uint8_t cnt8[BE_ITER][TPB];
	uint32_t n = 0;
	for (uint32_t it = 0; it < BE_ITER; it++) {
		const uint32_t S = S0 + it * TPB;
		const uint32_t p = S < nS ? side_tidx[S] : NIL;
		uint32_t k = 0;
		if (p != NIL) {
			uint32_t highest = NIL;
			k = side_back_edges<false, IC>(S, p, 0, loff, ladj, dps, side_tidx, ckey, voff, t_par, b_src, b_tgt, b_ord, dupflag, incnt, highest,
						   first2[it][threadIdx.x]);
			ordcnt[p] = (OC)k;
			hi0[p] = highest;
			n += k;
		}
		cnt8[it][threadIdx.x] = (uint8_t)min(k, 255u);
	}
	__shared__ uint32_t wsum[TPB / 64], base;
	uint32_t all;
	const uint32_t before = block_exclusive_scan<TPB / 64>(n, wsum, all, ScanOp<0>{});
	if (threadIdx.x == 0)
		base = all ? atomicAdd(total_out, all) : 0u;
	__syncthreads();
	if (!n || base + all > cap)
		return;
	uint32_t at = base + before;
	for (uint32_t it = 0; it < BE_ITER; it++) {
		const uint32_t k = cnt8[it][threadIdx.x];
		if (!k)
			continue;
		const uint32_t S = S0 + it * TPB, p = side_tidx[S];
		if (k <= 2) {
			uint32_t root = NIL;
			if constexpr (sizeof(IC) == 1) {
				const uint32_t c = ckey[S >> 1];
// ... 119 lines not shown
		if (groups & 1)
			spans(n, p...);
	};
	auto take = [&](size_t n, auto *&...p) {
		if (groups & 2)
			spans(n, p...);
	};
	const size_t nS = 2 * V + 2, NA = std::max<size_t>(4 * V, 2 * E) + 8;
	const size_t NSL = std::max<size_t>(2 * V + 2 * E, 4 * V) + 16;
	if (groups & 1)
		spans.bytes_for(tw.dvis_slots, std::max(2 * E, 2 * V) + 16);
	take1(nS, tw.side_tidx);
	take1(nS, tw.dps);
	take(2 * E + 16, tw.dist);
	take(NA / 64 + 4, tw.xrec);
	take(NA / 64 + 4, tw.xrank);
	if (groups & 2)
		spans.bytes_for(tw.evt, NA * 8);
	take(V + 2, tw.t0seg);
	take(nS, tw.entry_ps, tw.entry_list, tw.be_cnt);
	take(nS, tw.dvis);
	take(nS + 2 * E + 8, tw.wadj);
	take(Cmax + 2, tw.cproc);
	take(NSL, tw.rk_pk);
	take(Cmax + 2, tw.rk_heads);
	const size_t pool_b = Arena::padded(rank_pool_words(NSL, Cmax + 1), 4);
	const size_t xv_b = Arena::padded(std::max<size_t>(V + 2, E + 8) + 8, 16);
	const WalkBytes wb(nS);
	char *blk = nullptr;
	if (groups & 2)
		spans.bytes_for(blk, o.walk_inline ? std::max(6 * pool_b + 2 * xv_b, wb.total()) : 6 * pool_b + 2 * xv_b);
	if (groups & 2)
		tw.walk_inline = o.walk_inline;
	if (blk) {
		uint32_t **pools[6] = {&tw.rk_nx, &tw.rk_wa, &tw.rk_wb, &tw.rk_tA, &tw.rk_tB, &tw.rk_tC};
		for (int k = 0; k < 6; k++)
			*pools[k] = reinterpret_cast<uint32_t *>(blk + (size_t)k * pool_b);
		tw.xval = reinterpret_cast<decltype(tw.xval)>(blk + 6 * pool_b);
		tw.xps = reinterpret_cast<decltype(tw.xps)>(blk + 6 * pool_b + xv_b);
		if (o.walk_inline) {
			tw.wrec = reinterpret_cast<decltype(tw.wrec)>(blk);
			tw.wstk = reinterpret_cast<decltype(tw.wstk)>(blk + wb.rec);
			tw.wpar = reinterpret_cast<decltype(tw.wpar)>(blk + wb.rec + wb.stk);
		} else {
			tw.wrec = nullptr;
			tw.wstk = nullptr;
			tw.wpar = nullptr;
		}
	}
}

size_t tree_workspace_bytes(size_t V, size_t E, size_t Cmax, int groups, const StageWsOpts &o)
{
	TreeWs tmp{};
	return measure([&](Spans &take) { tree_spans(tmp, V, E, Cmax, groups, o, take); }) + (1 << 20);
}

void tree_carve(Arena &ar, TreeWs &tw, size_t V, size_t E, size_t Cmax, int groups, const StageWsOpts &o)
{
	Spans take{&ar};
	tree_spans(tw, V, E, Cmax, groups, o, take);
}

size_t walk_workspace_bytes(size_t V) { return WalkBytes(2 * V + 2).total() + 4096; }

size_t stage_workspace_bytes(size_t V, size_t E, size_t Cmax, const StageWsOpts &o)
{
	return par_workspace_bytes(V, E, Cmax, 1, o) + tree_workspace_bytes(V, E, Cmax, 1, o) +
	       std::max(tree_workspace_bytes(V, E, Cmax, 2, o), par_workspace_bytes(V, E, Cmax, 2, o));
}
void stage_workspace_carve(Arena &ar, ParWs &pw, TreeWs &tw, size_t V, size_t E, size_t Cmax, const StageWsOpts &o)
{
	par_carve(ar, pw, V, E, Cmax, 1, o);
	tree_carve(ar, tw, V, E, Cmax, 1, o);
	const size_t shared = ar.used();
	tree_carve(ar, tw, V, E, Cmax, 2, o);
	const size_t tree_end = ar.used();
	ar.rewind(shared);
	par_carve(ar, pw, V, E, Cmax, 2, o);
	ar.advance_to(tree_end);
}

struct TreeViews {
	ulonglong2 *hside;
	uint32_t *ft;
	uint2 *fstr;
	uint8_t *multi;
	uint32_t *cstate;
	uint8_t *merged;
	uint32_t *over_list;
	uint32_t *k1, *k2;
	uint32_t *v1, *v2;
	uint32_t *side_of;
};
static TreeViews tree_views(const TreeWs &tw, uint32_t E, uint32_t *cur = nullptr)
{
	const size_t n_slots = 2 * (size_t)E;
	TreeViews v;
	v.hside = reinterpret_cast<ulonglong2 *>(tw.evt);
	v.ft = tw.be_cnt;
	v.fstr = reinterpret_cast<uint2 *>(tw.rk_pk);
	v.multi = tw.dvis_slots;
	v.cstate = cur;
	v.merged = tw.dvis;
	v.over_list = tw.entry_ps;
	v.k1 = reinterpret_cast<uint32_t *>(tw.xval), v.k2 = v.k1 + n_slots;
	v.v1 = reinterpret_cast<uint32_t *>(tw.xps), v.v2 = v.v1 + n_slots;
	v.side_of = reinterpret_cast<uint32_t *>(tw.evt);
	return v;
}

void tree_tour_words(const CompState &cs, uint32_t V, uint32_t E, TreeWs &tw, bool force_sparse_splitters, hipStream_t s)
{
	const uint32_t nS = 2 * V;
	const size_t n_slots = 2 * (size_t)E;
	if (n_slots >= P0_END || 3 * (size_t)V >= P0_END)
		throw HipError("graph too large for the packed list ranking: 2 * links and 3 * segments must stay below 2^30");
	const unsigned bitsA = force_sparse_splitters ? 4u : rank_bucket_bits(n_slots);
	const TreeViews v = tree_views(tw, E);
	LAUNCH(k_tour_words, nS, s, nS, cs.loff, cs.ladj, cs.lle, tw.rk_pk, bitsA, v.hside, v.ft);
	tw.tour_words_done = true;
}

struct TreePass {
	const CompState &cs;
	SeqWs &sw;
	ParWs &pw;
	TreeWs &tw;
	StageTimer &tm;
	hipStream_t s;
	const uint32_t C, V, E, nS;
	const uint32_t max_side_links;
	const bool force_big_class_dfs, force_sparse_splitters;
	const TreeViews v;
	const unsigned long long *start_key;
	const uint32_t NA;
	const size_t n_slots;
	const uint32_t XW;
	const uint32_t n_events;
	const unsigned bitsA, bitsE;
	RankBufs rb;
	L0Ranks tour_r{}, evr{};
	bool events_done = false;
	const uint8_t *dupflag = nullptr;

	TreePass(const CompState &cs_, SeqWs &sw_, ParWs &pw_, TreeWs &tw_, uint32_t C_, uint32_t max_side_links_, bool big_dfs, bool sparse,
		 StageTimer &tm_, hipStream_t s_)
		: cs(cs_), sw(sw_), pw(pw_), tw(tw_), tm(tm_), s(s_), C(C_), V(sw_.V), E(sw_.E), nS(2 * sw_.V), max_side_links(max_side_links_),
		  force_big_class_dfs(big_dfs), force_sparse_splitters(sparse), v(tree_views(tw_, sw_.E, sw_.cur)),
		  start_key((const unsigned long long *)cs_.start_key), NA(2 * (V - C)), n_slots(2 * (size_t)E), XW(NA / 64 + 1), n_events(3 * V),
		  bitsA(sparse ? 4u : rank_bucket_bits(n_slots)), bitsE(sparse ? 4u : rank_bucket_bits(n_events)),
		  rb{tw_.rk_pk, tw_.rk_heads, tw_.rk_nx, tw_.rk_wa, tw_.rk_wb, tw_.rk_tA, tw_.rk_tB, tw_.rk_tC}
	{
	}
	void enqueue_events()
	{
		HIP_CHECK(hipMemsetAsync(rb.heads, 0xFF, (size_t)C * 4, s));
		LAUNCH(k_events, V, s, V, tw.dps, cs.loff, cs.ladj, cs.ckey, tw.cproc, rb.pk, rb.heads, bitsE, v.merged, pw.sdl);
	}
};

static void root_forest(TreePass &P)
{
	const CompState &cs = P.cs;
	TreeWs &tw = P.tw;
	hipStream_t s = P.s;
	const uint32_t V = P.V, C = P.C;
	P.tm.begin("tree_root_forest");
	if (!tw.tour_words_done)
		tree_tour_words(cs, V, P.E, tw, P.force_sparse_splitters, s);
	tw.tour_words_done = false;
	LAUNCH(k_tour_ends, C, s, C, cs.voff, P.start_key, cs.loff, cs.ladj, cs.lle, P.rb.pk, P.rb.heads);
	if (P.n_slots)
		P.tour_r = list_rank_splitters<false>((uint32_t)P.n_slots, P.bitsA, tw.dist, nullptr, C, P.rb, s);
	HIP_CHECK(hipMemsetAsync(tw.xrec, 0, ((size_t)P.XW + 2) * 16, s));
	LAUNCH(k_t0_parents, std::max(V, C), s, V, tw.dist, P.tour_r, cs.ckey, cs.voff, cs.loff, cs.ladj, cs.lle, P.v.ft, P.rb.heads,
	       tw.t0seg, P.v.fstr, tw.xrec, C, P.start_key, P.pw.err + PW_FOREST_SIZE, P.v.multi);
	P.tm.end(40);
}

static void bridges_and_classes(TreePass &P)
{
	const CompState &cs = P.cs;
	ParWs &pw = P.pw;
	TreeWs &tw = P.tw;
	const TreeViews &v = P.v;
	hipStream_t s = P.s;
	const uint32_t V = P.V, XW = P.XW;
	P.tm.begin("tree_bridges_classes");
	bitrank_build(tw.xrec, XW, tw.xrank, pw.scan_tmp, pw.scan_tmp_bytes, s);
	LAUNCH(k_tour_values, V, s, V, tw.t0seg, v.ft, v.hside, tw.xrec, tw.xval);
	scan_exclusive_xor_u128(tw.xval, tw.xps, (size_t)V + 1, pw.scan_tmp, pw.scan_tmp_bytes, s, tw.xrank + XW);
	LAUNCH(k_bridges, V, s, V, tw.t0seg, v.fstr, tw.xps, tw.xrec, v.hside, cs.loff, cs.lle, cs.ckey, tw.cproc, v.multi, v.cstate, tw.dps);
	P.tm.end(8 + 44);
}

static void walk_large_classes(TreePass &P, uint32_t n_big, const uint32_t *big_list)
{
	const CompState &cs = P.cs;
	ParWs &pw = P.pw;
	TreeWs &tw = P.tw;
	hipStream_t s = P.s;
	const uint32_t nS = P.nS;
	if (!tw.walk_inline) {
		if (!tw.walk_arena)
			throw HipError("class walk: no arena for the wave walk's arrays (internal)");
		const WalkBytes wb(2 * (size_t)P.V + 2);
		tw.walk_arena->reserve(walk_workspace_bytes(P.V));
		tw.wrec = reinterpret_cast<decltype(tw.wrec)>(tw.walk_arena->take<char>(wb.rec));
		tw.wstk = reinterpret_cast<decltype(tw.wstk)>(tw.walk_arena->take<char>(wb.stk));
		tw.wpar = reinterpret_cast<decltype(tw.wpar)>(tw.walk_arena->take<char>(wb.par));
	}
	uint32_t *pool_top = pw.err + PW_POOL_TOP, *walk_err = pw.err + PW_WALK_POOL;
	LAUNCH(k_class_recs, nS, s, nS, cs.loff, cs.ladj, P.v.cstate, cs.ckey, tw.cproc, tw.wadj, tw.wrec, tw.wpar);
	const uint32_t route = getenv("POVU_HIP_WALK_ROUTE") ? (uint32_t)atoi(getenv("POVU_HIP_WALK_ROUTE")) : 0u;
	const uint32_t pool_cap = (uint32_t)std::min<size_t>(3 * (size_t)nS, 0xFFFFFFF0u);
	hipStream_t s2 = tw.walk_stream ? tw.walk_stream : s;
	if (s2 != s) {
		HIP_CHECK(hipEventRecord(tw.walk_fork, s));
		HIP_CHECK(hipStreamWaitEvent(s2, tw.walk_fork, 0));
	}
	KLAUNCH(k_class_walk_wave<false>, dim3(n_big), dim3(64), 0, s2, n_big, big_list, tw.wrec, tw.wadj, tw.wpar, tw.wstk, pool_top, pool_cap,
		walk_err, nS, route);
	KLAUNCH(k_class_walk_wave<true>, dim3(n_big), dim3(64), 0, s, n_big, big_list, tw.wrec, tw.wadj, tw.wpar, tw.wstk, pool_top, pool_cap,
		walk_err, nS, route);
	if (s2 != s) {
		HIP_CHECK(hipEventRecord(tw.walk_join, s2));
		HIP_CHECK(hipStreamWaitEvent(s, tw.walk_join, 0));
	}
	LAUNCH(k_walk_finish, nS, s, nS, tw.wpar, P.v.cstate, cs.loff, cs.ladj, tw.dps);
	if (tw.host->read_u32(walk_err, s))
		throw HipError("class walk: stack pool exhausted (internal sizing bug)");
}

static void class_walks(TreePass &P)
{
	const CompState &cs = P.cs;
	ParWs &pw = P.pw;
	TreeWs &tw = P.tw;
	const TreeViews &v = P.v;
	hipStream_t s = P.s;
	const uint32_t nS = P.nS;
	P.tm.begin("tree_class_dfs");
	uint32_t *n_entry_dev = pw.err + PW_N_ENTRY;
	KLAUNCH(k_entry_list, dim3((nS + EL_SIDES - 1) / EL_SIDES), dim3(TPB), 0, s, nS, v.cstate, v.multi, cs.ckey, tw.cproc, tw.entry_list, n_entry_dev);
	const uint32_t *big_list = tw.entry_list;
	uint32_t n_big = P.force_big_class_dfs ? tw.host->read_u32(n_entry_dev, s) : 0;
	if (!P.force_big_class_dfs) {
		const unsigned all_blocks = (nS + 63) / 64;
		unsigned dfs_blocks = std::min(all_blocks, 49152u);
		if (const char *ev = getenv("POVU_HIP_DFS_BLOCKS"))
			dfs_blocks = std::min(all_blocks, std::max(1u, (unsigned)atoi(ev)));
		uint32_t *n_over = pw.err + PW_N_OVER;
		uint32_t budget = CLASS_BUDGET;
		if (const char *ev = getenv("POVU_HIP_CLASS_BUDGET"))
			budget = (uint32_t)std::max(16, atoi(ev));
		KLAUNCH(k_class_dfs_small, dim3(dfs_blocks), dim3(64), 0, s, n_entry_dev, tw.entry_list, cs.loff, cs.ladj, v.cstate, tw.dps,
			budget, n_over, v.over_list);
		if (!P.tm.enabled) {
			uint32_t *w = tw.host->take<uint32_t>(1);
			publish_words(w, WordSrc{{n_over}}, 1, s);
			const HostScratch::Token published = tw.host->mark(s);
			P.enqueue_events();
			tw.host->wait(published);
			n_big = *w;
			P.events_done = n_big == 0;
		} else {
			n_big = tw.host->read_u32(n_over, s);
		}
		big_list = v.over_list;
	}
	if (n_big)
		walk_large_classes(P, n_big, big_list);
	P.tm.end(5);
}

static void preorder(TreePass &P)
{
	P.tm.begin("tree_preorder");
	if (!P.events_done)
		P.enqueue_events();
	P.evr = list_rank_splitters<true, true>(P.n_events, P.bitsE, P.tw.evt, P.pw.err + PW_RANK_OVF, P.C, P.rb, P.s);
	P.tm.end(40);
}

static void emit_tree(TreePass &P)
{
	const CompState &cs = P.cs;
	SeqWs &sw = P.sw;
	ParWs &pw = P.pw;
	TreeWs &tw = P.tw;
	P.tm.begin("tree_emit");
	auto tree_emit = [&](auto *ordcnt, auto *srccnt, auto *incnt) {
		using OC = std::remove_pointer_t<decltype(ordcnt)>;
		using SC = std::remove_pointer_t<decltype(srccnt)>;
		using IC = std::remove_pointer_t<decltype(incnt)>;
		LAUNCH((k_tree_emit<OC, SC, IC>), std::max(P.V, P.C), P.s, P.nS, tw.evt, P.evr, P.v.merged, tw.dps, cs.ckey, tw.cproc, cs.voff, P.start_key, cs.gid_s, sw.t_gid,
		       sw.t_flags, sw.t_par, sw.t_size, (sw.hairpins || sw.want_depth) ? sw.t_depth : nullptr, tw.side_tidx, P.C, sw.c_ntree, ordcnt,
		       pw.hi0, pw.mpre, srccnt, pw.sdl, incnt);
	};
	if (pw.narrow_ordcnt && pw.narrow_srccnt && pw.narrow_incnt)
		tree_emit(pw.ordcnt8, pw.srccnt8, pw.incnt8);
	else if (pw.narrow_ordcnt && pw.narrow_srccnt)
		tree_emit(pw.ordcnt8, pw.srccnt8, pw.incnt);
	else if (pw.narrow_ordcnt)
		tree_emit(pw.ordcnt8, pw.dlt, pw.incnt);
	else
		tree_emit(pw.lsz, pw.dlt, pw.incnt);
	pw.sdl_filled = true;
}

static void dup_flags(TreePass &P)
{
	const CompState &cs = P.cs;
	ParWs &pw = P.pw;
	TreeWs &tw = P.tw;
	const TreeViews &v = P.v;
	hipStream_t s = P.s;
	if (P.max_side_links > 64 && P.E) {
		const uint32_t n_slots = 2 * P.E, nS = P.nS;
		LAUNCH(k_slot_keys, n_slots, s, n_slots, cs.ladj, v.k1, v.v1);
		sort_pairs_u32(v.k1, v.k2, v.v1, v.v2, n_slots, bits_for(nS), pw.sort_tmp, pw.sort_tmp_bytes, s);
		LAUNCH(k_slot_side, nS, s, nS, cs.loff, v.side_of);
		LAUNCH(k_gather_keys, n_slots, s, n_slots, v.v2, v.side_of, v.k1);
		sort_pairs_u32(v.k1, v.k2, v.v2, v.v1, n_slots, bits_for(nS), pw.sort_tmp, pw.sort_tmp_bytes, s);
		LAUNCH(k_dup_flags, n_slots, s, n_slots, v.k2, v.v1, cs.ladj, tw.dvis_slots);
		P.dupflag = tw.dvis_slots;
	}
	tw.last_dupflag = P.dupflag;
}

static void back_edges(TreePass &P)
{
	const CompState &cs = P.cs;
	ParWs &pw = P.pw;
	TreeWs &tw = P.tw;
	auto launch = [&](auto *ordcnt, auto *incnt) {
		KLAUNCH((k_back_edges<std::remove_pointer_t<decltype(ordcnt)>, std::remove_pointer_t<decltype(incnt)>>), dim3((P.nS + BE_SIDES - 1) / BE_SIDES), dim3(TPB), 0, P.s, P.nS, cs.loff, cs.ladj, tw.dps, tw.side_tidx, cs.ckey,
			cs.voff, P.sw.t_par, pw.err + PW_NB0, pw.b_src, pw.b_tgt, pw.b_ord, P.dupflag, ordcnt, pw.hi0, incnt,
			(uint32_t)std::min<size_t>(pw.nb_cap, 0xFFFFFFFFu));
	};
	if (pw.narrow_ordcnt && pw.narrow_srccnt && pw.narrow_incnt)
		launch(pw.ordcnt8, pw.incnt8);
	else if (pw.narrow_ordcnt)
		launch(pw.ordcnt8, pw.incnt);
	else
		launch(pw.lsz, pw.incnt);
	P.tm.end(6);
}

int64_t run_parallel_tree(const CompState &cs, SeqWs &sw, ParWs &pw, TreeWs &tw, uint32_t C, uint32_t max_side_links,
			   bool force_big_class_dfs, bool force_sparse_splitters, StageTimer &tm, hipStream_t s)
{
	TreePass P(cs, sw, pw, tw, C, max_side_links, force_big_class_dfs, force_sparse_splitters, tm, s);
	root_forest(P);
	bridges_and_classes(P);
	class_walks(P);
	preorder(P);
	emit_tree(P);
	dup_flags(P);
	back_edges(P);
	return NB0_ON_DEVICE;
}

}
```

povu_amd/csrc/hip/tree_kernels.hpp:

```cpp
#pragma once
#include "common.hpp"
#include "graph_kernels.hpp"
#include "par_kernels.hpp"
#include "seq_kernels.hpp"

namespace povu_hip
{

struct TreeWs {
	HostScratch *host;
	uint2 *dist;
	ulonglong2 *xval, *xps;
	uint4 *xrec;
	uint32_t *xrank;
	uint4 *t0seg;
	uint2 *dps;
	uint8_t *dvis;
	uint32_t *wadj;
	uint4 *wrec;
	uint2 *wstk;
	uint32_t *wpar;
	uint8_t *dvis_slots;
	uint32_t *entry_ps, *entry_list;
	uint32_t *side_tidx;
	uint32_t *be_cnt;
	uint32_t *rk_pk, *rk_heads;
	uint32_t *rk_nx, *rk_wa, *rk_wb, *rk_tA, *rk_tB, *rk_tC;
	uint2 *evt;
	uint32_t *cproc;
	const uint8_t *last_dupflag;
	bool tour_words_done = false;
	hipStream_t walk_stream = nullptr;
	hipEvent_t walk_fork = nullptr, walk_join = nullptr;
	Arena *walk_arena = nullptr;
	bool walk_inline = true;
};

size_t tree_workspace_bytes(size_t V, size_t E, size_t Cmax, int groups = 3, const StageWsOpts &o = StageWsOpts{});
void tree_carve(Arena &ar, TreeWs &tw, size_t V, size_t E, size_t Cmax, int groups = 3, const StageWsOpts &o = StageWsOpts{});
size_t stage_workspace_bytes(size_t V, size_t E, size_t Cmax, const StageWsOpts &o = StageWsOpts{});
void stage_workspace_carve(Arena &ar, ParWs &pw, TreeWs &tw, size_t V, size_t E, size_t Cmax, const StageWsOpts &o = StageWsOpts{});
size_t walk_workspace_bytes(size_t V);

void tree_tour_words(const CompState &cs, uint32_t V, uint32_t E, TreeWs &tw, bool force_sparse_splitters, hipStream_t s);

int64_t run_parallel_tree(const CompState &cs, SeqWs &sw, ParWs &pw, TreeWs &tw, uint32_t C, uint32_t max_side_links,
			   bool force_big_class_dfs, bool force_sparse_splitters, StageTimer &tm, hipStream_t s);

void debug_list_rank(uint32_t n, const uint32_t *next, const uint8_t *w, const uint32_t *heads, uint32_t nh, int mode,
		     unsigned bits, uint32_t *ra, uint32_t *rb, hipStream_t s);

void edge_id_weights(const CompState &cs, const SeqWs &sw, const TreeWs &tw, uint32_t *w, uint32_t *tail, hipStream_t s);

}
```

povu_amd/hip.py:

```python
from __future__ import annotations

import ctypes as C
import os
from dataclasses import dataclass
from typing import Dict, List, Optional

import numpy as np

_HERE = os.path.dirname(os.path.abspath(__file__))


class HipUnavailable(RuntimeError):
    pass


class GuardBandError(RuntimeError):
    """A device-wide primitive wrote outside its output (raised by its unit-test hook, which guards every output)."""


SCAN_SUM, SCAN_MAX, SCAN_U64, SCAN_U8, SCAN_DIFF, SCAN_XOR_PAIR, SCAN_XOR_U128, SCAN_DIFF_U8, SCAN_MIXED_PAIR, SCAN_DIFF_U8_U8 = range(10)
SCAN_IN_PLACE, SCAN_N_DEV = 0x100, 0x200
SEG_MIN, SEG_FIRST_LESS, SEG_LAST_LESS = range(3)


def lib_path() -> str:
    return os.path.join(_HERE, "lib", "libpovu_hip.so")


class _Opts(C.Structure):
    _fields_ = [("rank", C.c_uint32), ("world", C.c_uint32), ("flags", C.c_uint32)]


class _SubTree(C.Structure):
    _fields_ = [("n_total", C.c_uint32), ("n_flubble_like", C.c_uint32), ("n_concealed", C.c_uint32), ("n_midi", C.c_uint32),
                ("n_smothered", C.c_uint32), ("fam", C.POINTER(C.c_uint8)), ("or1", C.POINTER(C.c_uint8)),
                ("or2", C.POINTER(C.c_uint8)), ("route", C.POINTER(C.c_uint8)), ("id1", C.POINTER(C.c_uint32)),
                ("id2", C.POINTER(C.c_uint32)), ("child_off", C.POINTER(C.c_uint32)), ("child", C.POINTER(C.c_uint32))]


class _Tree(C.Structure):
    _fields_ = [("component_id", C.c_uint32), ("n_vtx", C.c_uint32), ("n_links", C.c_uint32),
                ("n_pvst", C.c_uint32), ("a_id", C.POINTER(C.c_uint32)), ("z_id", C.POINTER(C.c_uint32)),
                ("a_or", C.POINTER(C.c_uint8)), ("z_or", C.POINTER(C.c_uint8)), ("parent", C.POINTER(C.c_uint32)),
                ("n_hairpins", C.c_uint32), ("hairpins", C.POINTER(C.c_uint64))]


class _ShardInfo(C.Structure):
    _fields_ = [("n_vtx", C.c_uint32), ("n_links", C.c_uint32), ("n_components", C.c_uint32), ("weight", C.c_uint64),
                ("bytes", C.c_size_t), ("device_ptr", C.c_void_p)]


class _MultiRank(C.Structure):
    _fields_ = [("device", C.c_int), ("n_vtx", C.c_uint32), ("n_links", C.c_uint32), ("n_components", C.c_uint32),
                ("shard_bytes", C.c_uint64), ("recv_ms", C.c_double), ("csr_ms", C.c_double), ("decompose_ms", C.c_double),
                ("sink_ms", C.c_double), ("h2d", C.c_uint64), ("d2h", C.c_uint64), ("peer_out", C.c_uint64),
                ("peer_in", C.c_uint64)]


class _WalkOpts(C.Structure):
    _fields_ = [("max_walks", C.c_uint32), ("max_steps", C.c_uint32), ("max_expansions", C.c_uint32), ("flags", C.c_uint32)]


class _Walks(C.Structure):
    _fields_ = [("n_queries", C.c_uint64), ("n_walks", C.c_uint64), ("n_steps", C.c_uint64),
                ("walk_off", C.POINTER(C.c_uint32)), ("step_off", C.POINTER(C.c_uint32)), ("step_id", C.POINTER(C.c_uint32)),
                ("step_or", C.POINTER(C.c_uint8)), ("status", C.POINTER(C.c_uint8)), ("n_tier2", C.c_uint64),
                ("device_ms", C.c_double)]


class _TravOpts(C.Structure):
    _fields_ = [("max_steps", C.c_uint32), ("flags", C.c_uint32)]


class _Traversals(C.Structure):
    _fields_ = [("n_queries", C.c_uint64), ("n_traversals", C.c_uint64), ("n_alleles", C.c_uint64), ("n_steps", C.c_uint64),
                ("trav_off", C.POINTER(C.c_uint64)), ("allele_off", C.POINTER(C.c_uint64)), ("status", C.POINTER(C.c_uint8)),
                ("path", C.POINTER(C.c_uint32)), ("first", C.POINTER(C.c_uint32)), ("last", C.POINTER(C.c_uint32)),
                ("allele", C.POINTER(C.c_uint32)), ("reverse", C.POINTER(C.c_uint8)), ("step_off", C.POINTER(C.c_uint64)),
                ("step_id", C.POINTER(C.c_uint32)), ("step_or", C.POINTER(C.c_uint8)), ("n_tier2", C.c_uint64),
                ("n_hash_splits", C.c_uint64), ("device_ms", C.c_double)]


class _Sites(C.Structure):
    _fields_ = [("n", C.c_uint32), ("id1", C.POINTER(C.c_uint32)), ("id2", C.POINTER(C.c_uint32)), ("or1", C.POINTER(C.c_uint8)),
                ("or2", C.POINTER(C.c_uint8)), ("parent", C.POINTER(C.c_uint32)), ("height", C.POINTER(C.c_uint32)),
                ("family", C.POINTER(C.c_uint8)), ("tree", C.POINTER(C.c_uint32))]


class _CallRefs(C.Structure):
    _fields_ = [("n_refs", C.c_uint32), ("ref_path", C.POINTER(C.c_uint32)), ("n_slots", C.c_uint32), ("n_samples", C.c_uint32),
                ("sample_of_slot", C.POINTER(C.c_uint32))]


class _CallNames(C.Structure):
    _fields_ = [("refs", _CallRefs), ("n_paths", C.c_uint32), ("slot_of_path", C.POINTER(C.c_uint32)),
                ("sample", C.POINTER(C.c_char_p)), ("slot_hap", C.POINTER(C.c_int64))]


class _VcfDoc(C.Structure):
    _fields_ = ([(k, C.c_uint64) for k in ("n_samples", "n_records", "n_alleles", "n_steps", "n_text_bytes", "n_tasks", "n_id_bytes")] +
                [("sample", C.POINTER(C.c_char_p)), ("rec_line", C.POINTER(C.c_uint64)), ("rec_pos", C.POINTER(C.c_uint64)),
                 ("rec_id_off", C.POINTER(C.c_uint64)), ("ids", C.POINTER(C.c_uint8)), ("allele_off", C.POINTER(C.c_uint64)),
                 ("task_off", C.POINTER(C.c_uint64)), ("step_off", C.POINTER(C.c_uint64)), ("text_off", C.POINTER(C.c_uint64)),
                 ("allele_walk", C.POINTER(C.c_uint8)), ("step_id", C.POINTER(C.c_uint32)), ("step_or", C.POINTER(C.c_uint8)),
                 ("text", C.POINTER(C.c_uint8))] +
                [(k, C.POINTER(C.c_uint32)) for k in ("task_record", "task_allele", "task_col", "task_phase")])


class _VcfOpts(C.Structure):
    _fields_ = [("flags", C.c_uint32)]


class _VcfReport(C.Structure):
    _fields_ = ([(k, C.c_uint64) for k in ("n_records", "n_tasks", "n_alleles")] +
                [(k, C.POINTER(C.c_uint8)) for k in ("task_status", "allele_spell", "rec_invalid", "rec_reason")] +
                [(k, C.POINTER(C.c_uint32)) for k in ("rec_allele", "rec_task")] +
                [("n_status", C.c_uint64 * 6), ("n_invalid", C.c_uint64), ("n_misspelled", C.c_uint64), ("n_tier2", C.c_uint64),
                 ("device_ms", C.c_double)])


OFFREF_COUNTERS = ("n_offref_sites", "n_offref_records", "n_offref_hosted")
MERGE_COUNTERS = ("n_merged_groups", "n_merged_members", "n_merge_splits", "n_ref_consistent", "n_gt_conflicts")


class _Calls(C.Structure):
    _fields_ = ([(k, C.c_uint64) for k in ("n_records", "n_slots", "n_blocks", "n_spelled", "n_seq_bytes", "n_at_bytes", "n_refs")] +
                [(k, C.POINTER(C.c_uint32)) for k in ("query", "path", "first", "ref_allele", "n_alleles", "an", "ns", "block")] +
                [("pos", C.POINTER(C.c_uint64)), ("flags", C.POINTER(C.c_uint8)), ("ac_off", C.POINTER(C.c_uint64)),
                 ("ac", C.POINTER(C.c_uint32)), ("gt", C.POINTER(C.c_uint16)), ("block_off", C.POINTER(C.c_uint64)),
                 ("seq_off", C.POINTER(C.c_uint64)), ("at_off", C.POINTER(C.c_uint64)), ("seq", C.POINTER(C.c_uint8)),
                 ("at", C.POINTER(C.c_uint8)), ("contig_len", C.POINTER(C.c_uint64)), ("device_ms", C.c_double),
                 ("n_steps", C.POINTER(C.c_uint32))] +
                [(k, C.c_uint64) for k in ("n_inv_records", "n_inv_heads", "n_inv_long", "n_inv_tier2")])


class _CallsNested(_Calls):
    _fields_ = ([("level", C.POINTER(C.c_uint32)), ("parent_query", C.POINTER(C.c_uint32)), ("ref_spelled", C.POINTER(C.c_uint64))] +
                [(k, C.c_uint64) for k in ("n_enclosed", "n_collapsed_sites", "n_popped", "n_rescued", "nested")] +
                [("raw_pos", C.POINTER(C.c_uint64))] +
                [(k, C.POINTER(C.c_uint32)) for k in ("norm_block", "norm_shift", "norm_chop", "norm_trim")] +
                [(k, C.c_uint64) for k in ("n_normalized", "max_shift", "n_norm_compared")] +
                [("n_rows", C.c_uint64), ("row_record", C.POINTER(C.c_uint32)), ("row_alt", C.POINTER(C.c_uint32)),
                 ("row_kind", C.POINTER(C.c_uint8)), ("row_reason", C.POINTER(C.c_uint8)), ("row_index", C.POINTER(C.c_uint32)),
                 ("row_pos", C.POINTER(C.c_uint64))] +
                [(k, C.POINTER(C.c_uint32)) for k in ("row_ref_start", "row_ref_len", "row_alt_start", "row_alt_len")] +
                [("row_lead", C.POINTER(C.c_uint8))] +
                [(k, C.POINTER(C.c_uint32)) for k in ("row_ac", "row_an", "row_ns")] +
                [(k, C.c_uint64) for k in ("n_decomposed_alts", "n_passthrough_alts", "n_prim_tier2", "n_prim_cells")] +
                [("merged", C.c_uint64), ("n_mrows", C.c_uint64), ("mrow_off", C.POINTER(C.c_uint64)),
                 ("mrow_member", C.POINTER(C.c_uint32)), ("mrow_gt", C.POINTER(C.c_uint8))] +
                [(k, C.POINTER(C.c_uint32)) for k in ("mrow_ac", "mrow_an", "mrow_ns")] +
                [(k, C.c_uint64) for k in MERGE_COUNTERS] +
                [("offref", C.c_uint64), ("rec_offref", C.POINTER(C.c_uint8)), ("host_query", C.POINTER(C.c_uint32)),
                 ("host_allele", C.POINTER(C.c_uint32)), ("n_off_contigs", C.c_uint64), ("off_contig_path", C.POINTER(C.c_uint32)),
                 ("off_contig_len", C.POINTER(C.c_uint64))] +
                [(k, C.c_uint64) for k in OFFREF_COUNTERS])


class _ProfileOpts(C.Structure):
    _fields_ = [("profile", C.c_uint32), ("max_level", C.c_uint32), ("max_ref_length", C.c_uint64),
                ("max_allele_length", C.c_uint64)]


class _StageTime(C.Structure):
    _fields_ = [("name", C.c_char * 48), ("ms", C.c_double), ("launches", C.c_uint32)]


F_HAIRPINS = 1
F_SEQUENTIAL = 2
F_SEQ_TREE = 4
F_FORCE_REDO = 8
F_SORTED_ADJ = 16
F_NO_STAGE_TIMES = 32
F_BIG_CLASS_DFS = 64
F_SPARSE_SPLITTERS = 128
F_REDO_ODD = 256
F_ALL_VERTEX_CLASSES = 512
F_CHECK_LAMINAR = 1024
F_LEAF_SUBFLUBBLES = 2048
F_ASYNC = 4096
F_SUBFLUBBLES = 8192

W_FORCE_TIER2 = 1
# ... 7 lines not shown
PROFILES = {"raw-graph": 0, "top-level-only": 1, "popped": 2, "left-normalized": 3, "decomposed": 4}
PRIM_MAX_LENGTH = 512
ROW_RAW, ROW_SNP, ROW_INS, ROW_DEL, ROW_PASS = 0, 1, 2, 3, 4
REASON_NONE, REASON_MAX_ALLELE_LENGTH, REASON_CONTIG_START, REASON_EMPTY_ALLELE, REASON_EQUALS_REF, REASON_SUBR = 0, 1, 2, 3, 4, 5

V_FOUND_FWD, V_FOUND_REV, V_ABSENT, V_NO_AT, V_BAD_STEP, V_NO_SLOT, V_MISSPELLED = range(7)
V_STATUS_NAMES = ("found_fwd", "found_rev", "absent", "no_at", "bad_step", "no_slot", "misspelled")
V_SPELL_NONE, V_SPELL_WHOLE, V_SPELL_ANCHORED, V_SPELL_MISSPELLED = range(4)
V_FORWARD_ONLY, V_SPELLING, V_FORCE_TIER2 = 1, 2, 4

_lib = None


def load_lib():
    global _lib
    if _lib is not None:
        return _lib
    p = lib_path()
    if not os.path.exists(p):
        raise HipUnavailable(f"{p} is missing: build it with `python -c 'import __graft_entry__ as g; g.build()'` "
                             "(there is no CPU fallback)")
    l = C.CDLL(p)
    l.povu_hip_device_count.restype = C.c_int
    l.povu_hip_create.restype = C.c_void_p
    l.povu_hip_create.argtypes = [C.c_int, C.c_char_p, C.c_size_t]
    l.povu_hip_destroy.argtypes = [C.c_void_p]
    l.povu_hip_graph_upload.restype = C.c_int
    l.povu_hip_graph_upload.argtypes = [C.c_void_p, C.c_uint32, C.c_void_p, C.c_uint32, C.c_void_p, C.c_void_p,
                                        C.c_void_p, C.c_void_p, C.c_void_p, C.c_char_p, C.c_size_t]
    l.povu_hip_last_upload_times.restype = C.c_int
    l.povu_hip_last_upload_times.argtypes = [C.c_void_p, C.POINTER(C.c_double)]
    l.povu_hip_decompose.restype = C.c_void_p
    l.povu_hip_decompose.argtypes = [C.c_void_p, C.POINTER(_Opts), C.c_char_p, C.c_size_t]
    l.povu_hip_forest_total_components.restype = C.c_uint32
    l.povu_hip_forest_total_components.argtypes = [C.c_void_p]
    l.povu_hip_forest_tree_count.restype = C.c_uint32
    l.povu_hip_forest_tree_count.argtypes = [C.c_void_p]
    l.povu_hip_forest_get.restype = C.c_int
    l.povu_hip_forest_get.argtypes = [C.c_void_p, C.c_uint32, C.POINTER(_Tree)]
    l.povu_hip_forest_free.argtypes = [C.c_void_p]
    l.povu_hip_forest_wait.restype = C.c_int
    l.povu_hip_forest_wait.argtypes = [C.c_void_p]
    l.povu_hip_forest_pass_ms.restype = C.c_double
    l.povu_hip_forest_pass_ms.argtypes = [C.c_void_p]
    l.povu_hip_forest_span_ms.restype = C.c_double
    l.povu_hip_forest_span_ms.argtypes = [C.c_void_p, C.c_void_p]
    l.povu_hip_forest_get_subtree.restype = C.c_int
    l.povu_hip_forest_get_subtree.argtypes = [C.c_void_p, C.c_uint32, C.c_void_p]
    l.povu_hip_forest_get_sub.restype = C.c_int
    l.povu_hip_forest_get_sub.argtypes = [C.c_void_p, C.c_uint32, C.POINTER(C.POINTER(C.c_uint32)),
                                          C.POINTER(C.POINTER(C.c_uint32)), C.POINTER(C.POINTER(C.c_uint8))]
    l.povu_hip_forest_raw.restype = C.c_int
    l.povu_hip_forest_raw.argtypes = [C.c_void_p, C.POINTER(C.c_void_p), C.POINTER(C.c_size_t), C.POINTER(C.c_uint64),
                                      C.POINTER(C.c_uint64)]
    l.povu_hip_forest_walks.restype = C.POINTER(_Walks)
    l.povu_hip_forest_walks.argtypes = [C.c_void_p, C.c_void_p, C.POINTER(_WalkOpts), C.c_char_p, C.c_size_t]
    l.povu_hip_walks_free.argtypes = [C.POINTER(_Walks)]
    l.povu_hip_paths_upload.restype = C.c_int
    l.povu_hip_paths_upload.argtypes = [C.c_void_p, C.c_uint32, C.c_void_p, C.c_void_p, C.c_void_p, C.c_char_p, C.c_size_t]
    l.povu_hip_forest_traversals.restype = C.POINTER(_Traversals)
    l.povu_hip_forest_traversals.argtypes = [C.c_void_p, C.c_void_p, C.POINTER(_TravOpts), C.c_char_p, C.c_size_t]
    l.povu_hip_traversals_free.argtypes = [C.POINTER(_Traversals)]
    l.povu_hip_forest_first.restype = C.c_uint64
    l.povu_hip_segments_upload.argtypes = [C.c_void_p, C.c_uint32, C.c_void_p, C.c_void_p, C.c_char_p, C.c_size_t]
    l.povu_hip_segments_upload.restype = C.c_int
    l.povu_hip_call.argtypes = [C.c_void_p, C.POINTER(_Sites), C.POINTER(_CallRefs), C.POINTER(C.c_uint32), C.POINTER(_TravOpts),
                                C.c_char_p, C.c_size_t]
    l.povu_hip_call.restype = C.POINTER(_CallsNested)
    l.povu_hip_call_profile.argtypes = [C.c_void_p, C.POINTER(_Sites), C.POINTER(_CallRefs), C.POINTER(C.c_uint32), C.POINTER(_TravOpts),
                                        C.POINTER(_ProfileOpts), C.c_char_p, C.c_size_t]
    l.povu_hip_call_profile.restype = C.POINTER(_CallsNested)
    l.povu_hip_calls_vcf_profile.argtypes = [C.POINTER(_CallsNested), C.POINTER(_Sites), C.POINTER(_CallNames), C.POINTER(C.c_char_p),
                                             C.c_char_p, C.c_char_p, C.c_uint32, C.c_uint32, C.POINTER(C.c_size_t)]
    l.povu_hip_calls_vcf_profile.restype = C.c_void_p
    l.povu_hip_calls_vcf_rest.argtypes = [C.POINTER(_CallsNested), C.POINTER(_Sites), C.POINTER(_CallNames), C.POINTER(C.c_char_p),
                                          C.c_char_p, C.POINTER(C.c_char_p), C.c_uint32, C.c_uint32, C.c_uint32, C.POINTER(C.c_size_t)]
    l.povu_hip_calls_vcf_rest.restype = C.c_void_p
    l.povu_hip_calls_free.argtypes = [C.POINTER(_Calls)]
    l.povu_hip_call_names_make.argtypes = [C.c_uint32, C.POINTER(C.c_char_p), C.c_uint32, C.POINTER(C.c_char_p), C.c_char_p,
                                           C.c_size_t]
    l.povu_hip_call_names_make.restype = C.POINTER(_CallNames)
    l.povu_hip_call_names_free.argtypes = [C.POINTER(_CallNames)]
    l.povu_hip_sites_of_docs.argtypes = [C.c_void_p, C.c_uint32]
    l.povu_hip_sites_of_docs.restype = C.POINTER(_Sites)
    l.povu_hip_forest_sites.argtypes = [C.c_void_p]
    l.povu_hip_forest_sites.restype = C.POINTER(_Sites)
    l.povu_hip_sites_free.argtypes = [C.POINTER(_Sites)]
    l.povu_hip_calls_vcf.argtypes = [C.POINTER(_Calls), C.POINTER(_Sites), C.POINTER(_CallNames), C.POINTER(C.c_char_p), C.c_char_p,
                                     C.c_char_p, C.c_uint32, C.POINTER(C.c_size_t)]
    l.povu_hip_calls_vcf.restype = C.c_void_p
    l.povu_hip_forest_first.argtypes = [C.c_void_p, C.c_uint32]
    l.povu_hip_vcf_parse.argtypes = [C.c_char_p, C.c_size_t, C.c_uint32, C.c_char_p, C.c_size_t]
    l.povu_hip_vcf_parse.restype = C.POINTER(_VcfDoc)
    l.povu_hip_vcf_doc_free.argtypes = [C.POINTER(_VcfDoc)]
    l.povu_hip_vcf_names_make.argtypes = [C.c_uint32, C.POINTER(C.c_char_p), C.c_char_p, C.c_size_t]
    l.povu_hip_vcf_names_make.restype = C.POINTER(_CallNames)
    l.povu_hip_vcf_columns.argtypes = [C.POINTER(_VcfDoc), C.POINTER(_CallNames), C.c_void_p, C.c_void_p]
    l.povu_hip_vcf_columns.restype = C.c_int
    l.povu_hip_vcf_check.argtypes = [C.c_void_p, C.POINTER(_VcfDoc), C.POINTER(_CallNames), C.POINTER(_VcfOpts), C.c_char_p, C.c_size_t]
    l.povu_hip_vcf_check.restype = C.POINTER(_VcfReport)
    l.povu_hip_vcf_report_free.argtypes = [C.POINTER(_VcfReport)]
    l.povu_hip_vcf_report_text.argtypes = [C.POINTER(_VcfReport), C.POINTER(_VcfDoc), C.POINTER(_CallNames), C.POINTER(C.c_size_t),
                                           C.POINTER(C.c_void_p), C.POINTER(C.c_size_t)]
    l.povu_hip_vcf_report_text.restype = C.c_void_p
    l.povu_hip_forest_pvst_text.restype = C.c_void_p
    l.povu_hip_forest_pvst_text.argtypes = [C.c_void_p, C.c_uint32, C.POINTER(C.c_size_t)]
    l.povu_hip_buffer_free.argtypes = [C.c_void_p]
    l.povu_hip_last_stage_times.restype = C.c_int
    l.povu_hip_last_stage_times.argtypes = [C.c_void_p, C.POINTER(_StageTime), C.c_int]
    l.povu_hip_last_seq_redo.restype = C.c_uint32
    l.povu_hip_last_seq_redo.argtypes = [C.c_void_p]
    l.povu_hip_last_links_processed.restype = C.c_uint64
    l.povu_hip_last_links_processed.argtypes = [C.c_void_p]
    l.povu_hip_debug_components.restype = C.c_int
    l.povu_hip_debug_components.argtypes = [C.c_void_p, C.c_void_p, C.c_void_p]
    l.povu_hip_debug_tree.restype = C.c_int
    l.povu_hip_debug_tree.argtypes = [C.c_void_p, C.c_uint32, C.POINTER(C.c_uint32), C.c_void_p, C.c_void_p,
                                      C.c_void_p, C.c_void_p]
    l.povu_hip_last_narrow_counts.restype = C.c_int
    l.povu_hip_last_narrow_counts.argtypes = [C.c_void_p]
    l.povu_hip_wide_repeats.restype = C.c_uint64
    l.povu_hip_wide_repeats.argtypes = [C.c_void_p]
    l.povu_hip_last_black_only_classes.restype = C.c_int
    l.povu_hip_last_black_only_classes.argtypes = [C.c_void_p]
    l.povu_hip_last_crossings.restype = C.c_int
    l.povu_hip_last_crossings.argtypes = [C.c_void_p, C.POINTER(C.c_uint32)]
    l.povu_hip_last_laminar_check_ran.restype = C.c_int
    l.povu_hip_last_laminar_check_ran.argtypes = [C.c_void_p]
    l.povu_hip_debug_edge_ids.restype = C.c_int
    l.povu_hip_debug_edge_ids.argtypes = [C.c_void_p, C.c_uint32, C.POINTER(C.c_uint32), C.c_void_p]
    l.povu_hip_debug_walk_words.restype = C.c_int
    l.povu_hip_debug_walk_words.argtypes = [C.c_void_p, C.POINTER(C.c_uint32)]
    l.povu_hip_debug_stack.restype = C.c_int
    l.povu_hip_debug_stack.argtypes = [C.c_void_p, C.c_uint32, C.POINTER(C.c_uint32), C.c_void_p, C.c_void_p,
                                       C.c_void_p]
    l.povu_hip_version.restype = C.c_char_p
    l.povu_hip_debug_scan.restype = C.c_int
    l.povu_hip_debug_scan.argtypes = [C.c_void_p, C.c_int, C.c_void_p, C.c_void_p, C.c_size_t, C.c_void_p, C.c_void_p,
                                      C.c_size_t]
    l.povu_hip_debug_sort.restype = C.c_int
    l.povu_hip_debug_sort.argtypes = [C.c_void_p, C.c_void_p, C.c_void_p, C.c_size_t, C.c_uint, C.c_void_p, C.c_void_p]
    l.povu_hip_debug_compact.restype = C.c_int
    l.povu_hip_debug_compact.argtypes = [C.c_void_p, C.c_void_p, C.c_size_t, C.c_void_p, C.POINTER(C.c_uint32)]
    l.povu_hip_debug_totals.restype = C.c_int
    l.povu_hip_debug_totals.argtypes = [C.c_void_p, C.c_void_p, C.c_void_p, C.c_size_t, C.POINTER(C.c_uint64)]
    l.povu_hip_debug_segtree.restype = C.c_int
    l.povu_hip_debug_segtree.argtypes = [C.c_void_p, C.c_void_p, C.c_size_t, C.c_void_p, C.c_size_t, C.c_void_p, C.c_void_p,
                                         C.POINTER(C.c_uint32)]
    l.povu_hip_debug_bitrank.restype = C.c_int
    l.povu_hip_debug_bitrank.argtypes = [C.c_void_p, C.c_void_p, C.c_size_t, C.c_void_p, C.c_size_t, C.c_void_p, C.c_void_p,
                                         C.c_void_p]
    l.povu_hip_debug_append.restype = C.c_int
    l.povu_hip_debug_append.argtypes = [C.c_void_p, C.c_void_p, C.c_size_t, C.c_void_p, C.POINTER(C.c_uint32)]
    l.povu_hip_debug_list_rank.restype = C.c_int
    l.povu_hip_debug_list_rank.argtypes = [C.c_void_p, C.c_uint32, C.c_void_p, C.c_void_p, C.c_void_p, C.c_uint32,
                                           C.c_int, C.c_uint32, C.c_void_p, C.c_void_p]
    l.povu_hip_workspace_estimate.restype = C.c_uint64
    l.povu_hip_workspace_estimate.argtypes = [C.c_uint32, C.c_uint32, C.c_uint32]
    l.povu_hip_prewarm.restype = C.c_int
    l.povu_hip_prewarm.argtypes = [C.c_void_p, C.c_uint32, C.c_uint32, C.c_char_p, C.c_size_t]
    l.povu_hip_leaf_workspace_estimate.restype = C.c_uint64
    l.povu_hip_leaf_workspace_estimate.argtypes = [C.c_uint32, C.c_uint32]
    l.povu_hip_lpt_assign.restype = C.c_int
    l.povu_hip_lpt_assign.argtypes = [C.c_void_p, C.c_uint32, C.c_uint32, C.c_void_p]
    l.povu_hip_shard_partition.restype = C.c_void_p
    l.povu_hip_shard_partition.argtypes = [C.c_void_p, C.c_uint32, C.c_char_p, C.c_size_t]
    l.povu_hip_shards_world.restype = C.c_uint32
    l.povu_hip_shards_world.argtypes = [C.c_void_p]
    l.povu_hip_shards_total_components.restype = C.c_uint32
    l.povu_hip_shards_total_components.argtypes = [C.c_void_p]
    l.povu_hip_shards_get.restype = C.c_int
    l.povu_hip_shards_get.argtypes = [C.c_void_p, C.c_uint32, C.POINTER(_ShardInfo)]
    l.povu_hip_shards_times.restype = C.c_int
    l.povu_hip_shards_times.argtypes = [C.c_void_p, C.POINTER(C.c_double)]
    l.povu_hip_shards_export.restype = C.c_int
    l.povu_hip_shards_export.argtypes = [C.c_void_p, C.c_void_p, C.c_uint32, C.c_void_p]
    l.povu_hip_shards_free.argtypes = [C.c_void_p]
    l.povu_hip_graph_upload_shard.restype = C.c_int
    l.povu_hip_graph_upload_shard.argtypes = [C.c_void_p, C.c_void_p, C.c_size_t, C.c_int, C.c_char_p, C.c_size_t]
    l.povu_hip_shard_total_components.restype = C.c_uint32
    l.povu_hip_shard_total_components.argtypes = [C.c_void_p]
    l.povu_hip_forest_globalize.restype = C.c_int
    l.povu_hip_forest_globalize.argtypes = [C.c_void_p, C.c_void_p]
    l.povu_hip_forest_pack_size.restype = C.c_size_t
    l.povu_hip_forest_pack_size.argtypes = [C.c_void_p]
    l.povu_hip_forest_pack.restype = C.c_int
    l.povu_hip_forest_pack.argtypes = [C.c_void_p, C.c_void_p, C.c_size_t]
    l.povu_hip_forest_merge.restype = C.c_void_p
    l.povu_hip_forest_merge.argtypes = [C.c_void_p, C.POINTER(C.c_void_p), C.POINTER(C.c_size_t), C.c_uint32, C.c_char_p,
                                        C.c_size_t]
    l.povu_hip_comm_unique_id.restype = C.c_int
    l.povu_hip_comm_unique_id.argtypes = [C.c_char_p, C.c_char_p, C.c_size_t]
    l.povu_hip_comm_create.restype = C.c_void_p
    l.povu_hip_comm_create.argtypes = [C.c_void_p, C.c_char_p, C.c_uint32, C.c_uint32, C.c_char_p, C.c_size_t]
    l.povu_hip_comm_destroy.argtypes = [C.c_void_p]
    l.povu_hip_comm_scatter.restype = C.c_int
    l.povu_hip_comm_scatter.argtypes = [C.c_void_p, C.c_void_p, C.c_void_p, C.c_char_p, C.c_size_t]
    l.povu_hip_comm_gather.restype = C.c_void_p
    l.povu_hip_comm_gather.argtypes = [C.c_void_p, C.c_void_p, C.c_char_p, C.c_size_t]
    l.povu_hip_comm_times.restype = C.c_int
    l.povu_hip_comm_times.argtypes = [C.c_void_p, C.POINTER(C.c_double)]
    l.povu_hip_share_results.restype = C.c_int
    l.povu_hip_share_results.argtypes = [C.c_void_p, C.c_char_p, C.c_char_p, C.c_size_t]
    l.povu_hip_forest_share.restype = C.c_int
    l.povu_hip_forest_share.argtypes = [C.c_void_p, C.POINTER(C.c_uint64)]
    l.povu_hip_forest_attach.restype = C.c_void_p
    l.povu_hip_forest_attach.argtypes = [C.c_void_p, C.c_void_p, C.c_uint32, C.c_char_p, C.c_void_p, C.c_uint32, C.c_char_p,
                                         C.c_size_t]
    l.povu_hip_transfer_bytes.restype = C.c_int
    l.povu_hip_transfer_bytes.argtypes = [C.c_void_p, C.POINTER(C.c_uint64)]
    l.povu_hip_multi_create.restype = C.c_void_p
    l.povu_hip_multi_create.argtypes = [C.POINTER(C.c_int), C.c_uint32, C.c_char_p, C.c_size_t]
    l.povu_hip_multi_destroy.argtypes = [C.c_void_p]
    l.povu_hip_multi_world.restype = C.c_uint32
    l.povu_hip_multi_world.argtypes = [C.c_void_p]
    l.povu_hip_multi_upload.restype = C.c_int
    l.povu_hip_multi_upload.argtypes = [C.c_void_p, C.c_uint32, C.c_void_p, C.c_uint32, C.c_void_p, C.c_void_p, C.c_void_p,
                                        C.c_void_p, C.c_void_p, C.c_char_p, C.c_size_t]
    l.povu_hip_multi_scatter.restype = C.c_int
    l.povu_hip_multi_scatter.argtypes = [C.c_void_p, C.c_int, C.c_char_p, C.c_size_t]
    l.povu_hip_multi_decompose.restype = C.c_void_p
    l.povu_hip_multi_decompose.argtypes = [C.c_void_p, C.c_uint32, C.c_void_p, C.c_void_p, C.c_char_p, C.c_size_t]
    l.povu_hip_multi_rank.restype = C.c_int
    l.povu_hip_multi_rank.argtypes = [C.c_void_p, C.c_uint32, C.POINTER(_MultiRank)]
    l.povu_hip_multi_times.restype = C.c_int
    l.povu_hip_multi_times.argtypes = [C.c_void_p, C.POINTER(C.c_double)]
    l.povu_hip_multi_transport.restype = C.c_char_p
    l.povu_hip_multi_transport.argtypes = [C.c_void_p]
    l.povu_hip_gfa_write.restype = C.c_int
    l.povu_hip_gfa_write.argtypes = [C.c_char_p, C.c_uint32, C.c_void_p, C.c_uint32, C.c_void_p, C.c_void_p, C.c_void_p,
                                     C.c_void_p, C.c_char_p, C.c_size_t]
    _lib = l
    return l


def write_gfa(links, path: str) -> None:
    l = load_lib()
    vid = np.ascontiguousarray(links.vid, dtype=np.uint32)
    v1 = np.ascontiguousarray(links.v1, dtype=np.uint32)
    v2 = np.ascontiguousarray(links.v2, dtype=np.uint32)
    s1 = np.ascontiguousarray(links.s1, dtype=np.uint8)
    s2 = np.ascontiguousarray(links.s2, dtype=np.uint8)
    err = C.create_string_buffer(512)
    if l.povu_hip_gfa_write(path.encode(), len(vid), vid.ctypes.data, len(v1), v1.ctypes.data, s1.ctypes.data,
                            v2.ctypes.data, s2.ctypes.data, err, 512) != 0:
        raise RuntimeError(err.value.decode())


def lpt_assign(weights, world: int) -> np.ndarray:
    w = np.ascontiguousarray(weights, dtype=np.uint64)
    out = np.zeros(len(w), dtype=np.uint32)
    if load_lib().povu_hip_lpt_assign(w.ctypes.data, len(w), world, out.ctypes.data) != 0:
        raise ValueError("bad LPT arguments")
    return out


@dataclass
class PvstTree:
    component_id: int
    n_vtx: int
    n_links: int
    a_id: np.ndarray
    z_id: np.ndarray
    a_or: np.ndarray
    z_or: np.ndarray
    parent: np.ndarray
    hairpins: np.ndarray
    text: Optional[str] = None


class Forest:

    def __init__(self, lib, handle):
        self._lib, self._h = lib, handle

    def __del__(self):
        if getattr(self, "_h", None):
            self._lib.povu_hip_forest_free(self._h)
            self._h = None

    def wait(self) -> "Forest":
        self._lib.povu_hip_forest_wait(self._h)
        return self

    def pass_ms(self) -> float:
        return float(self._lib.povu_hip_forest_pass_ms(self._h))

    def span_ms(self, last: "Forest") -> float:
        return float(self._lib.povu_hip_forest_span_ms(self._h, last._h))

    @property
    def total_components(self) -> int:
        return self._lib.povu_hip_forest_total_components(self._h)

    def __len__(self) -> int:
        return self._lib.povu_hip_forest_tree_count(self._h)

    def pvst_sizes(self) -> List[int]:
        out = []
        t = _Tree()
        for i in range(len(self)):
            if self._lib.povu_hip_forest_get(self._h, i, C.byref(t)) != 0:
                raise IndexError(i)
            out.append(int(t.n_pvst))
        return out

# ... 695 lines not shown
        self._prim_rc(rc, "scan_exclusive_u32_pair" if op == 0 else name)
        return out, out2

    def debug_scan_u8(self, a, b=None):
        a = np.ascontiguousarray(a, dtype=np.uint8)
        out = np.empty(a.size, dtype=np.uint32)
        if b is None:
            rc = self._lib.povu_hip_debug_scan(self._ctx, SCAN_U8, a.ctypes.data, out.ctypes.data, a.size, None, None, 0)
            self._prim_rc(rc, "scan_exclusive_u8")
            return out
        b = np.ascontiguousarray(b, dtype=np.uint8)
        out2 = np.empty(b.size, dtype=np.uint32)
        rc = self._lib.povu_hip_debug_scan(self._ctx, SCAN_U8, a.ctypes.data, out.ctypes.data, a.size, b.ctypes.data,
                                           out2.ctypes.data, b.size)
        self._prim_rc(rc, "scan_exclusive_u8 (two jobs)")
        return out, out2

    def debug_scan_diff(self, a, sub):
        a = np.ascontiguousarray(a, dtype=np.uint32)
        sub = np.ascontiguousarray(sub, dtype=np.uint32)
        assert a.size == sub.size
        out = np.empty_like(a)
        rc = self._lib.povu_hip_debug_scan(self._ctx, SCAN_DIFF, a.ctypes.data, out.ctypes.data, a.size, sub.ctypes.data,
                                           None, sub.size)
        self._prim_rc(rc, "scan_exclusive_diff_u32")
        return out

    def debug_scan_diff_u8(self, a, sub):
        a = np.ascontiguousarray(a, dtype=np.uint8)
        sub = np.ascontiguousarray(sub, dtype=np.uint32)
        assert a.size == sub.size
        out = np.empty(a.size, dtype=np.uint32)
        rc = self._lib.povu_hip_debug_scan(self._ctx, SCAN_DIFF_U8, a.ctypes.data, out.ctypes.data, a.size, sub.ctypes.data,
                                           None, sub.size)
        self._prim_rc(rc, "scan_exclusive_diff_u8_u32")
        return out

    def debug_scan_diff_u8_u8(self, a, sub):
        a = np.ascontiguousarray(a, dtype=np.uint8)
        sub = np.ascontiguousarray(sub, dtype=np.uint8)
        assert a.size == sub.size
        out = np.empty(a.size, dtype=np.uint32)
        rc = self._lib.povu_hip_debug_scan(self._ctx, SCAN_DIFF_U8_U8, a.ctypes.data, out.ctypes.data, a.size, sub.ctypes.data,
                                           None, sub.size)
        self._prim_rc(rc, "scan_exclusive_diff_u8_u8")
        return out

    def debug_scan_mixed_pair(self, a, b):
        a = np.ascontiguousarray(a, dtype=np.uint32)
        b = np.ascontiguousarray(b, dtype=np.uint8)
        out, out2 = np.empty_like(a), np.empty(b.size, dtype=np.uint32)
        rc = self._lib.povu_hip_debug_scan(self._ctx, SCAN_MIXED_PAIR, a.ctypes.data, out.ctypes.data, a.size, b.ctypes.data,
                                           out2.ctypes.data, b.size)
        self._prim_rc(rc, "scan_exclusive_u32_u8_pair")
        return out, out2

    def debug_scan_xor_pair(self, a, b):
        a = np.ascontiguousarray(a, dtype=np.uint32)
        b = np.ascontiguousarray(b, dtype=np.uint32)
        assert a.size == b.size
        out, out2 = np.empty_like(a), np.empty_like(b)
        rc = self._lib.povu_hip_debug_scan(self._ctx, SCAN_XOR_PAIR, a.ctypes.data, out.ctypes.data, a.size,
                                           b.ctypes.data, out2.ctypes.data, b.size)
        self._prim_rc(rc, "scan_exclusive_xor_u32_pair")
        return out, out2

    def debug_scan_xor_u128(self, a, n_dev=None):
        a = np.ascontiguousarray(a, dtype=np.uint64)
        assert a.ndim == 2 and a.shape[1] == 2
        out = np.empty_like(a)
        op = SCAN_XOR_U128 | (SCAN_N_DEV if n_dev is not None else 0)
        rc = self._lib.povu_hip_debug_scan(self._ctx, op, a.ctypes.data, out.ctypes.data, a.shape[0], None, None,
                                           n_dev or 0)
        self._prim_rc(rc, "scan_exclusive_xor_u128")
        return out if n_dev is None else out[:min(n_dev + 1, a.shape[0])]

    def debug_sort(self, keys, vals, bits: int):
        keys = np.ascontiguousarray(keys, dtype=np.uint32)
        vals = np.ascontiguousarray(vals, dtype=np.uint32)
        assert keys.size == vals.size
        ko, vo = np.empty_like(keys), np.empty_like(vals)
        rc = self._lib.povu_hip_debug_sort(self._ctx, keys.ctypes.data, vals.ctypes.data, keys.size, bits,
                                           ko.ctypes.data, vo.ctypes.data)
        self._prim_rc(rc, "sort_pairs_u32")
        return ko, vo

    def debug_compact(self, flags):
        flags = np.ascontiguousarray(flags, dtype=np.uint8)
        out = np.empty(flags.size, dtype=np.uint32)
        cnt = C.c_uint32(0)
        rc = self._lib.povu_hip_debug_compact(self._ctx, flags.ctypes.data, flags.size, out.ctypes.data, C.byref(cnt))
        self._prim_rc(rc, "compact_flagged_u8")
        if cnt.value > flags.size:
            raise RuntimeError(f"compact_flagged_u8: count {cnt.value} of {flags.size} flags")
        return out[:cnt.value], int(cnt.value)

    def debug_totals(self, a, b=None):
        a = np.ascontiguousarray(a, dtype=np.uint32)
        tot = (C.c_uint64 * 2)()
        if b is not None:
            b = np.ascontiguousarray(b, dtype=np.uint32)
            assert a.size == b.size
        rc = self._lib.povu_hip_debug_totals(self._ctx, a.ctypes.data, b.ctypes.data if b is not None else None, a.size, tot)
        self._prim_rc(rc, "totals_u32")
        return int(tot[0]) if b is None else (int(tot[0]), int(tot[1]))

    def debug_segtree(self, values, queries, want_tree: bool = False):
        values = np.ascontiguousarray(values, dtype=np.uint32)
        queries = np.ascontiguousarray(queries, dtype=np.uint32).reshape(-1, 4)
        out = np.empty(queries.shape[0], dtype=np.uint32)
        P = 1
        while P * 16 < values.size:
            P *= 2
        tree = np.empty(2 * P, dtype=np.uint32) if want_tree else None
        p_dev = C.c_uint32(0)
        rc = self._lib.povu_hip_debug_segtree(self._ctx, values.ctypes.data, values.size, queries.ctypes.data, queries.shape[0],
                                              out.ctypes.data, tree.ctypes.data if want_tree else None, C.byref(p_dev))
        self._prim_rc(rc, "segment tree (seg_build / seg_min / seg_first_less / seg_last_less)")
        if p_dev.value != P:
            raise RuntimeError(f"segment tree: P = {p_dev.value} for {values.size} values, {P} expected")
        return (out, tree, P) if want_tree else out

    def debug_bitrank(self, flags, positions):
        flags = np.ascontiguousarray(flags, dtype=np.uint8)
        positions = np.ascontiguousarray(positions, dtype=np.uint32)
        rank, test = np.empty(positions.size, dtype=np.uint32), np.empty(positions.size, dtype=np.uint32)
        records = np.empty((flags.size // 64 + 2, 4), dtype=np.uint32)
        rc = self._lib.povu_hip_debug_bitrank(self._ctx, flags.ctypes.data, flags.size, positions.ctypes.data, positions.size,
                                              rank.ctypes.data, test.ctypes.data, records.ctypes.data)
        self._prim_rc(rc, "bit-rank directory (bitrank_store_wave / bitrank_build)")
        return rank, test, records

    def debug_append(self, flags):
        flags = np.ascontiguousarray(flags, dtype=np.uint8)
        out = np.empty(flags.size, dtype=np.uint32)
        cnt = C.c_uint32(0)
        rc = self._lib.povu_hip_debug_append(self._ctx, flags.ctypes.data, flags.size, out.ctypes.data, C.byref(cnt))
        self._prim_rc(rc, "append_in_order")
        if cnt.value > flags.size:
            raise RuntimeError(f"append_in_order: length {cnt.value} of {flags.size} flags")
        return out[:cnt.value], int(cnt.value)

    def debug_list_rank(self, nxt, w, heads, events: bool = False, bits: int = 0):
        nxt = np.ascontiguousarray(nxt, dtype=np.uint32)
        w = np.ascontiguousarray(w, dtype=np.uint8)
        heads = np.ascontiguousarray(heads, dtype=np.uint32)
        ra = np.zeros(nxt.size, dtype=np.uint32)
        rb = np.zeros(nxt.size, dtype=np.uint32)
        rc = self._lib.povu_hip_debug_list_rank(self._ctx, nxt.size, nxt.ctypes.data, w.ctypes.data,
                                                heads.ctypes.data if heads.size else None, heads.size,
                                                1 if events else 0, bits, ra.ctypes.data, rb.ctypes.data)
        if rc:
            raise RuntimeError(f"debug_list_rank failed ({rc})")
        return (ra, rb) if events else ra

    def debug_components(self, n_vtx: int):
        comp = np.zeros(n_vtx, dtype=np.uint32)
        loc = np.zeros(n_vtx, dtype=np.uint32)
        if self._lib.povu_hip_debug_components(self._ctx, comp.ctypes.data, loc.ctypes.data) != 0:
            raise RuntimeError("no decompose state")
        return comp, loc

    def debug_tree(self, comp: int):
        n = C.c_uint32(0)
        if self._lib.povu_hip_debug_tree(self._ctx, comp, C.byref(n), None, None, None, None) != 0:
            raise RuntimeError("no decompose state")
        gid = np.zeros(n.value, dtype=np.uint32)
        typ = np.zeros(n.value, dtype=np.uint8)
        par = np.zeros(n.value, dtype=np.uint32)
        cls = np.zeros(n.value, dtype=np.uint32)
        self._lib.povu_hip_debug_tree(self._ctx, comp, C.byref(n), gid.ctypes.data, typ.ctypes.data, par.ctypes.data,
                                      cls.ctypes.data)
        return dict(gid=gid, typ=typ & 3, black=(typ >> 2) & 1, root=(typ >> 3) & 1, par=par, cls=cls)

    def last_narrow_counts(self) -> bool:
        return bool(self._lib.povu_hip_last_narrow_counts(self._ctx))

    def last_narrow_forms(self) -> tuple:
        m = int(self._lib.povu_hip_last_narrow_counts(self._ctx))
        return bool(m & 1), bool(m & 2), bool(m & 4)

    def wide_repeat_count(self) -> int:
        return int(self._lib.povu_hip_wide_repeats(self._ctx))

    def last_black_only_classes(self) -> bool:
        return bool(self._lib.povu_hip_last_black_only_classes(self._ctx))

    def last_crossings(self):
        o = (C.c_uint32 * 2)()
        if self._lib.povu_hip_last_crossings(self._ctx, o) != 0:
            raise RuntimeError("povu_hip_last_crossings failed")
        return int(o[0]), int(o[1])

    def last_laminar_check_ran(self) -> bool:
        return bool(self._lib.povu_hip_last_laminar_check_ran(self._ctx))

    def debug_edge_ids(self, comp: int):
        n = C.c_uint32(0)
        rc = self._lib.povu_hip_debug_edge_ids(self._ctx, comp, C.byref(n), None)
        if rc != 0:
            raise RuntimeError("no parallel-tree state" if rc == 3 else "no decompose state")
        ids = np.zeros(n.value, dtype=np.uint32)
        if self._lib.povu_hip_debug_edge_ids(self._ctx, comp, C.byref(n), ids.ctypes.data) != 0:
            raise RuntimeError("povu_hip_debug_edge_ids failed")
        return ids

    def debug_walk_words(self):
        o = (C.c_uint32 * 3)()
        rc = self._lib.povu_hip_debug_walk_words(self._ctx, o)
        if rc != 0:
            raise RuntimeError("no parallel-tree state" if rc in (3, 4) else "no decompose state")
        return dict(n_entry=int(o[0]), n_over=int(o[1]), pool_top=int(o[2]))

    def debug_stack(self, comp: int):
        n = C.c_uint32(0)
        if self._lib.povu_hip_debug_stack(self._ctx, comp, C.byref(n), None, None, None) != 0:
            raise RuntimeError("no decompose state")
        vtx = np.zeros(n.value, dtype=np.uint32)
        cls = np.zeros(n.value, dtype=np.uint32)
        ns = np.zeros(n.value, dtype=np.uint32)
        self._lib.povu_hip_debug_stack(self._ctx, comp, C.byref(n), vtx.ctypes.data, cls.ctypes.data, ns.ctypes.data)
        return dict(tree_vtx=vtx, cls=cls, next_seen=ns)


class MultiDecomposer:

    def __init__(self, devices):
        self._lib = load_lib()
        if self._lib.povu_hip_device_count() <= 0:
            raise HipUnavailable("no HIP device visible: the decompose path has no CPU fallback")
        devs = (C.c_int * len(devices))(*[int(d) for d in devices])
        err = C.create_string_buffer(512)
        self._h = self._lib.povu_hip_multi_create(devs, len(devices), err, 512)
        if not self._h:
            raise HipUnavailable(err.value.decode())
        self.world = len(devices)

    def close(self):
        if getattr(self, "_h", None):
            self._lib.povu_hip_multi_destroy(self._h)
            self._h = None

    def __del__(self):
        self.close()

    @property
    def transport(self) -> str:
        return self._lib.povu_hip_multi_transport(self._h).decode()

    def upload(self, links, tips=None):
        vid = np.ascontiguousarray(links.vid, dtype=np.uint32)
        v1 = np.ascontiguousarray(links.v1, dtype=np.uint32)
        v2 = np.ascontiguousarray(links.v2, dtype=np.uint32)
        s1 = np.ascontiguousarray(links.s1, dtype=np.uint8)
        s2 = np.ascontiguousarray(links.s2, dtype=np.uint8)
        tp = None
        if tips is not None:
            tips = np.ascontiguousarray(tips, dtype=np.uint8)
            tp = tips.ctypes.data
        err = C.create_string_buffer(512)
        if self._lib.povu_hip_multi_upload(self._h, len(vid), vid.ctypes.data, len(v1), v1.ctypes.data, s1.ctypes.data,
                                           v2.ctypes.data, s2.ctypes.data, tp, err, 512) != 0:
            raise RuntimeError(err.value.decode())

    def scatter(self, keep_graph: bool = True):
        err = C.create_string_buffer(512)
        if self._lib.povu_hip_multi_scatter(self._h, 1 if keep_graph else 0, err, 512) != 0:
            raise RuntimeError(err.value.decode())

    def decompose(self, flags: int = 0) -> Forest:
        err = C.create_string_buffer(512)
        h = self._lib.povu_hip_multi_decompose(self._h, flags, None, None, err, 512)
        if not h:
            raise RuntimeError(err.value.decode())
        return Forest(self._lib, h)

    def rank_info(self, rank: int) -> dict:
        r = _MultiRank()
        if self._lib.povu_hip_multi_rank(self._h, rank, C.byref(r)) != 0:
            raise IndexError(rank)
        return {k: getattr(r, k) for k, _ in _MultiRank._fields_}

    def times(self) -> dict:
        t = (C.c_double * 6)()
        self._lib.povu_hip_multi_times(self._h, t)
        return dict(label_ms=t[0], lpt_ms=t[1], partition_ms=t[2], scatter_wall_ms=t[3], decompose_wall_ms=t[4], merge_ms=t[5])
```

Measured before the change: 3.365 billion.

## Compress list-rank records into a 32-bit plane with escape fallback plane

Replaces the 8-byte uint2 per-element rank record with a split layout: a 32-bit primary word packing a signed owner delta relative to the bucket plus small partial ranks, and a second word plane read only when an escape bit is set. Readers in resolve, t0_parents and tree_emit load the primary plane and fetch the second plane only when a lane in the wavefront needs it, with the aim of halving record memory traffic. It also adds an env-gated debug statistics kernel and API for measuring escape rates. This costs extra encode/decode arithmetic and a branch, and throughput depends on how often records escape.

```diff
diff --git a/include/povu_hip.h b/include/povu_hip.h
--- a/include/povu_hip.h
+++ b/include/povu_hip.h
@@ -496,6 +496,16 @@
 int povu_hip_debug_append(povu_hip_ctx *ctx, const uint8_t *flags, size_t n, uint32_t *list, uint32_t *count);
 int povu_hip_debug_list_rank(povu_hip_ctx *ctx, uint32_t n, const uint32_t *next, const uint8_t *w, const uint32_t *heads,
 			     uint32_t nh, int mode, uint32_t bits, uint32_t *ra, uint32_t *rb);
+typedef struct povu_hip_rank_records {
+	uint64_t live;
+	uint64_t escaped;
+	uint32_t final_ranks;
+	uint32_t bucket_bits;
+	uint32_t delta_bits;
+	uint32_t partial_bits[2];
+	uint64_t hist[33 * 33];
+} povu_hip_rank_records;
+int povu_hip_debug_rank_escapes(povu_hip_ctx *ctx, int which, povu_hip_rank_records *out, uint8_t *esc, size_t n_esc);
 double povu_hip_debug_scan_time(povu_hip_ctx *ctx, size_t n, int reps, int op);
 
 uint64_t povu_hip_workspace_estimate(uint32_t n_vtx, uint32_t n_links, uint32_t n_components);
diff --git a/povu_amd/csrc/hip/context.hpp b/povu_amd/csrc/hip/context.hpp
--- a/povu_amd/csrc/hip/context.hpp
+++ b/povu_amd/csrc/hip/context.hpp
@@ -229,6 +229,8 @@
 	ParWs pw{};
 	TreeWs tw{};
 	LastPass last;
+	RankRecStats dbg_rank_stats;
+	std::vector<uint32_t> dbg_rank_plane0;
 	std::vector<uint32_t> shard_comp_ids;
 	uint32_t shard_total_components = 0;
 	Arena shard_buf;
diff --git a/povu_amd/csrc/hip/debug_hooks.hip b/povu_amd/csrc/hip/debug_hooks.hip
--- a/povu_amd/csrc/hip/debug_hooks.hip
+++ b/povu_amd/csrc/hip/debug_hooks.hip
@@ -422,11 +422,37 @@
 		return 1;
 	try {
 		HIP_CHECK(hipSetDevice(ctx->device));
-		debug_list_rank(n, next, w, heads, nh, mode, bits, ra, rb, ctx->stream);
-		return 0;
-	} catch (const std::exception &) {
-		return 2;
-	}
+		ctx->dbg_rank_stats.valid = false;
+		debug_list_rank(n, next, w, heads, nh, mode, bits, ra, rb, ctx->stream, &ctx->dbg_rank_stats, &ctx->dbg_rank_plane0);
+		return 0;
+	} catch (const std::exception &) {
+		return 2;
+	}
+}
+
+extern "C" int povu_hip_debug_rank_escapes(povu_hip_ctx *ctx, int which, povu_hip_rank_records *out, uint8_t *esc, size_t n_esc)
+{
+	if (!ctx || !out || which < 0 || which > 2 || (esc && which != 2))
+		return 1;
+	if (which < 2 && !ctx->last.valid)
+		return 1;
+	const RankRecStats &st = which == 2 ? ctx->dbg_rank_stats : ctx->tw.rec_stats[which];
+	if (!st.valid)
+		return 3;
+	if (esc && n_esc != ctx->dbg_rank_plane0.size())
+		return 1;
+	out->live = st.live;
+	out->escaped = st.esc;
+	out->final_ranks = st.fin;
+	out->bucket_bits = st.bits;
+	out->delta_bits = st.delta_bits;
+	out->partial_bits[0] = st.part_bits[0];
+	out->partial_bits[1] = st.part_bits[1];
+	std::copy(st.hist, st.hist + 33 * 33, out->hist);
+	if (esc)
+		for (size_t x = 0; x < n_esc; x++)
+			esc[x] = st.fin ? 1 : (uint8_t)(ctx->dbg_rank_plane0[x] >> 31);
+	return 0;
 }
 
 extern "C" double povu_hip_debug_scan_time(povu_hip_ctx *ctx, size_t n, int reps, int op)
diff --git a/povu_amd/csrc/hip/tree_kernels.hip b/povu_amd/csrc/hip/tree_kernels.hip
--- a/povu_amd/csrc/hip/tree_kernels.hip
+++ b/povu_amd/csrc/hip/tree_kernels.hip
@@ -272,10 +272,46 @@
 	}
 }
 static constexpr uint32_t REC_MAX = 0xFFFFu;
+static constexpr uint32_t REC_ESC = 0x80000000u;
+static constexpr unsigned REC_T_PBITS = 15, REC_T_DBITS = 16;
+static constexpr unsigned REC_E_PBITS = 7, REC_E_DBITS = 16;
+struct RecPlanes {
+	uint32_t *w0, *w1;
+};
+static RecPlanes rec_planes(uint2 *rec, size_t n)
+{
+	uint32_t *w = reinterpret_cast<uint32_t *>(rec);
+	return RecPlanes{w, w + ((n + 3) & ~(size_t)3)};
+}
+template <bool TWO>
+__device__ __forceinline__ void rec_store(const RecPlanes &rec, uint32_t x, unsigned b, uint32_t owner, uint32_t y)
+{
+	constexpr unsigned PB = TWO ? REC_E_PBITS : REC_T_PBITS, DB = TWO ? REC_E_DBITS : REC_T_DBITS;
+	constexpr uint32_t PMAX = (1u << PB) - 1u, HALF = 1u << (DB - 1);
+	const uint32_t d = owner - (x >> b), pa = TWO ? (y & REC_MAX) : y, pd = TWO ? (y >> 16) : 0u;
+	if (d + HALF < 2u * HALF && pa <= PMAX && pd <= PMAX) {
+		rec.w0[x] = ((d & (2u * HALF - 1u)) << (31u - DB)) | pa | (pd << PB);
+	} else {
+		rec.w0[x] = REC_ESC | owner;
+		rec.w1[x] = y;
+	}
+}
+template <bool TWO>
+__device__ __forceinline__ uint2 rec_decode(uint32_t x, unsigned b, uint32_t w0, uint32_t w1, bool fin = false)
+{
+	constexpr unsigned PB = TWO ? REC_E_PBITS : REC_T_PBITS, DB = TWO ? REC_E_DBITS : REC_T_DBITS;
+	constexpr uint32_t PMAX = (1u << PB) - 1u;
+	if (fin)
+		return make_uint2(w0, w1);
+	if (w0 & REC_ESC)
+		return make_uint2(w0 & ~REC_ESC, w1);
+	const uint32_t d = (uint32_t)((int32_t)(w0 << 1) >> (32 - DB));
+	return make_uint2((x >> b) + d, TWO ? ((w0 & PMAX) | (((w0 >> PB) & PMAX) << 16)) : (w0 & PMAX));
+}
 template <bool L0, bool TWO, bool EVT3 = false>
 __global__ void k_rank_up(RankLevelArgs A, unsigned b, const uint32_t *__restrict__ nx_in, const uint32_t *__restrict__ a_in,
 			  const uint32_t *__restrict__ b_in, const uint32_t *__restrict__ heads, uint32_t *__restrict__ nx_out,
-			  uint32_t *__restrict__ a_out, uint32_t *__restrict__ b_out, uint2 *__restrict__ rec, uint32_t *__restrict__ ovf)
+			  uint32_t *__restrict__ a_out, uint32_t *__restrict__ b_out, RecPlanes rec, uint32_t *__restrict__ ovf)
 {
 	const uint32_t id = BIDX * blockDim.x + threadIdx.x;
 	if (id >= A.M)
@@ -293,9 +329,9 @@
 				rank_l0_weights<EVT3>(x, p, wa, wb);
 				if (TWO) {
 					big |= sa > REC_MAX || sa - sb > REC_MAX;
-					rec[x] = make_uint2(id, sa | ((sa - sb) << 16));
+					rec_store<true>(rec, x, b, id, sa | ((sa - sb) << 16));
 				} else {
-					rec[x] = make_uint2(id, sa);
+					rec_store<false>(rec, x, b, id, sa);
 				}
 				sa += wa;
 				if (TWO)
@@ -324,7 +360,7 @@
 }
 template <bool EVT3>
 __global__ void k_rank_l0_fallback(RankLevelArgs A, unsigned b, const uint32_t *__restrict__ pk, const uint32_t *__restrict__ heads,
-				   const uint32_t *__restrict__ ra, const uint32_t *__restrict__ rb, uint2 *__restrict__ rec,
+				   const uint32_t *__restrict__ ra, const uint32_t *__restrict__ rb, RecPlanes rec,
 				   const uint32_t *__restrict__ ovf)
 {
 	if (!*ovf)
@@ -338,7 +374,8 @@
 			const uint32_t p = pk[x];
 			uint32_t wa, wb;
 			rank_l0_weights<EVT3>(x, p, wa, wb);
-			rec[x] = make_uint2(sa, sb);
+			rec.w0[x] = sa;
+			rec.w1[x] = sb;
 			sa -= wa;
 			sb -= wb;
 			x = p & P0_END;
@@ -436,6 +473,8 @@
 struct L0Ranks {
 	const uint32_t *ra, *rb, *fin;
 	uint32_t M;
+	const uint32_t *w0, *w1;
+	unsigned b;
 };
 __device__ __forceinline__ uint32_t l0_at(const L0Ranks &R, uint2 rec, bool want = true) { return want && rec.x < R.M ? rec.x : 0u; }
 __device__ __forceinline__ uint32_t rank_l0(const L0Ranks &R, uint2 rec, uint32_t ra) { return (rec.x < R.M ? ra : 0u) - rec.y; }
@@ -449,16 +488,93 @@
 	const uint32_t pa = rec.y & REC_MAX;
 	return fin ? rec : make_uint2((in ? ra : 0u) - pa, (in ? rb : 0u) - pa + (rec.y >> 16));
 }
-__device__ __forceinline__ uint32_t rank_l0(const L0Ranks &R, uint2 rec) { return rank_l0(R, rec, R.ra[l0_at(R, rec)]); }
-__device__ __forceinline__ uint2 rank_l0_pair(const L0Ranks &R, uint2 rec, bool fin)
-{
+__device__ __forceinline__ uint32_t rank_l0_of(const L0Ranks &R, uint32_t x)
+{
+	const uint32_t w0 = R.w0[x];
+	const uint2 rec = rec_decode<false>(x, R.b, w0, (w0 & REC_ESC) ? R.w1[x] : 0u);
+	return rank_l0(R, rec, R.ra[l0_at(R, rec)]);
+}
+__device__ __forceinline__ uint2 rank_l0_pair_of(const L0Ranks &R, uint32_t x, bool fin)
+{
+	const uint32_t w0 = R.w0[x];
+	const uint2 rec = rec_decode<true>(x, R.b, w0, (fin || (w0 & REC_ESC)) ? R.w1[x] : 0u, fin);
 	const uint32_t i = l0_at(R, rec, !fin);
 	return rank_l0_pair(R, rec, fin, R.ra[i], R.rb[i]);
 }
 
+__device__ __forceinline__ uint32_t bit_width(uint32_t v) { return 32u - (uint32_t)__clz(v); }
+template <bool TWO, bool EVT3>
+__global__ void k_rank_rec_stats(RankLevelArgs A, unsigned b, const uint32_t *__restrict__ pk, const uint32_t *__restrict__ heads,
+				 const uint32_t *__restrict__ w0, unsigned long long *__restrict__ out)
+{
+	__shared__ uint32_t h[2 + 33 * 33];
+	for (uint32_t i = threadIdx.x; i < 2 + 33 * 33; i += blockDim.x)
+		h[i] = 0;
+	__syncthreads();
+	for (uint32_t id = blockIdx.x * blockDim.x + threadIdx.x; id < A.M; id += gridDim.x * blockDim.x) {
+		uint32_t x = rank_lane_start<true>(id, A, b, pk, heads);
+		if (x == NIL)
+			continue;
+		uint32_t sa = 0, sb = 0;
+		do {
+			const uint32_t p = pk[x];
+			uint32_t wa, wb;
+			rank_l0_weights<EVT3>(x, p, wa, wb);
+			const int32_t d = (int32_t)(id - (x >> b));
+			const uint32_t zz = ((uint32_t)d << 1) ^ (uint32_t)(d >> 31);
+			const uint32_t pw = TWO ? max(bit_width(sa), bit_width(sa - sb)) : bit_width(sa);
+			atomicAdd(&h[0], 1u);
+			if (w0[x] & REC_ESC)
+				atomicAdd(&h[1], 1u);
+			atomicAdd(&h[2 + 33 * bit_width(zz) + pw], 1u);
+			sa += wa;
+			if (TWO)
+				sb += wb;
+			x = p & P0_END;
+		} while (!rank_l0_stop(x, b));
+	}
+	__syncthreads();
+	for (uint32_t i = threadIdx.x; i < 2 + 33 * 33; i += blockDim.x)
+		if (h[i])
+			atomicAdd(&out[i], (unsigned long long)h[i]);
+}
+template <bool TWO, bool EVT3>
+static void rank_rec_stats(const RankLevelArgs &A, unsigned b, const RankBufs &rb, const L0Ranks &R, RankRecStats &st, hipStream_t s)
+{
+	constexpr size_t W = 2 + 33 * 33;
+	st = RankRecStats{};
+	unsigned long long *d = nullptr;
+	uint32_t fin = 0;
+	std::vector<unsigned long long> hst(W);
+	HIP_CHECK(hipMalloc(reinterpret_cast<void **>(&d), W * 8));
+	try {
+		HIP_CHECK(hipMemsetAsync(d, 0, W * 8, s));
+		KLAUNCH((k_rank_rec_stats<TWO, EVT3>), dim3(std::min(nblk(A.M), 2048u)), dim3(TPB), 0, s, A, b, rb.pk, rb.heads, R.w0, d);
+		HIP_CHECK(copy_async(hst.data(), d, W * 8, hipMemcpyDeviceToHost, s));
+		if (TWO)
+			HIP_CHECK(copy_async(&fin, R.fin, 4, hipMemcpyDeviceToHost, s));
+		HIP_CHECK(hipStreamSynchronize(s));
+	} catch (...) {
+		(void)hipFree(d);
+		throw;
+	}
+	HIP_CHECK(hipFree(d));
+	st.valid = true;
+	st.fin = fin;
+	st.bits = b;
+	st.delta_bits = TWO ? REC_E_DBITS : REC_T_DBITS;
+	st.part_bits[0] = TWO ? REC_E_PBITS : REC_T_PBITS;
+	st.part_bits[1] = TWO ? REC_E_PBITS : 0u;
+	st.live = hst[0];
+	st.esc = fin ? hst[0] : hst[1];
+	std::copy(hst.begin() + 2, hst.end(), st.hist);
+}
+
 template <bool TWO, bool EVT3 = false>
-static L0Ranks list_rank_splitters(uint32_t n, unsigned b, uint2 *rec, uint32_t *ovf, uint32_t nh, RankBufs &rb, hipStream_t s)
-{
+static L0Ranks list_rank_splitters(uint32_t n, unsigned b, uint2 *rec_arr, uint32_t *ovf, uint32_t nh, RankBufs &rb, hipStream_t s,
+				   RankRecStats *st = nullptr)
+{
+	const RecPlanes rec = rec_planes(rec_arr, n);
 	if (n >= P0_END)
 		throw HipError("list ranking: more than 2^30 elements (graph too large for the packed walk)");
 	RankLevelArgs lv[RANK_MAX_LEVELS];
@@ -495,7 +611,7 @@
 			LAUNCH((k_rank_up<true, TWO, EVT3>), A.M, s, A, b, nxp[0], nullptr, nullptr, rb.heads, nxp[1], wap[1], wbp[1], rec, ovf);
 		else
 			LAUNCH((k_rank_up<false, TWO>), A.M, s, A, b, nxp[L], wap[L], wbp[L], nullptr, nxp[L + 1], wap[L + 1], wbp[L + 1],
-			       nullptr, nullptr);
+			       RecPlanes{nullptr, nullptr}, nullptr);
 	}
 	const uint32_t nt = cur_n;
 	if (nt <= RANK_TOP) {
@@ -520,25 +636,28 @@
 	if (TWO)
 		KLAUNCH((k_rank_l0_fallback<EVT3>), dim3(std::min(nblk(lv[0].M), 2048u)), dim3(TPB), 0, s, lv[0], b, rb.pk, rb.heads, wap[1],
 			wbp[1], rec, ovf);
-	return L0Ranks{wap[1], TWO ? wbp[1] : nullptr, TWO ? ovf : nullptr, lv[0].M};
+	const L0Ranks R{wap[1], TWO ? wbp[1] : nullptr, TWO ? ovf : nullptr, lv[0].M, rec.w0, rec.w1, b};
+	if (st)
+		rank_rec_stats<TWO, EVT3>(lv[0], b, rb, R, *st, s);
+	return R;
 }
 
 template <bool TWO>
-__global__ void k_rank_resolve(uint32_t n, const uint2 *__restrict__ rec, L0Ranks R, uint32_t *__restrict__ ra, uint32_t *__restrict__ rb)
+__global__ void k_rank_resolve(uint32_t n, L0Ranks R, uint32_t *__restrict__ ra, uint32_t *__restrict__ rb)
 {
 	const uint32_t x = BIDX * blockDim.x + threadIdx.x;
 	if (x >= n)
 		return;
 	if (TWO) {
-		const uint2 r = rank_l0_pair(R, rec[x], *R.fin != 0);
+		const uint2 r = rank_l0_pair_of(R, x, *R.fin != 0);
 		ra[x] = r.x;
 		rb[x] = r.y;
 	} else {
-		ra[x] = rank_l0(R, rec[x]);
+		ra[x] = rank_l0_of(R, x);
 	}
 }
 void debug_list_rank(uint32_t n, const uint32_t *next, const uint8_t *w, const uint32_t *heads, uint32_t nh, int mode,
-		     unsigned bits, uint32_t *ra, uint32_t *rb, hipStream_t s)
+		     unsigned bits, uint32_t *ra, uint32_t *rb, hipStream_t s, RankRecStats *st, std::vector<uint32_t> *plane0)
 {
 	if (n == 0 || n >= P0_END)
 		throw HipError("debug_list_rank: n must be in [1, 2^30)");
@@ -569,11 +688,15 @@
 	if (nh)
 		HIP_CHECK(copy_async(rbf.heads, heads, (size_t)nh * 4, hipMemcpyHostToDevice, s));
 	if (mode == 0) {
-		const L0Ranks R = list_rank_splitters<false>(n, b, rec, nullptr, nh, rbf, s);
-		LAUNCH(k_rank_resolve<false>, n, s, n, rec, R, da, nullptr);
+		const L0Ranks R = list_rank_splitters<false>(n, b, rec, nullptr, nh, rbf, s, st);
+		LAUNCH(k_rank_resolve<false>, n, s, n, R, da, nullptr);
 	} else {
-		const L0Ranks R = list_rank_splitters<true, true>(n, b, rec, ovf, nh, rbf, s);
-		LAUNCH(k_rank_resolve<true>, n, s, n, rec, R, da, db);
+		const L0Ranks R = list_rank_splitters<true, true>(n, b, rec, ovf, nh, rbf, s, st);
+		LAUNCH(k_rank_resolve<true>, n, s, n, R, da, db);
+	}
+	if (plane0) {
+		plane0->resize(n);
+		HIP_CHECK(copy_async(plane0->data(), rec, (size_t)n * 4, hipMemcpyDeviceToHost, s));
 	}
 	HIP_CHECK(copy_async(ra, da, (size_t)n * 4, hipMemcpyDeviceToHost, s));
 	if (mode != 0)
@@ -583,7 +706,7 @@
 
 static constexpr uint32_t T0_RBIT = 0x80000000u;
 static constexpr uint32_t BS_POS = 0x3FFFFFFFu, BS_NOARC = 0x80000000u, BS_HASH_L = 0x40000000u, BS_HASH_R = 0x80000000u;
-__global__ void k_t0_parents(uint32_t V, const uint2 *__restrict__ trec, L0Ranks R, const uint32_t *__restrict__ ckey,
+__global__ void k_t0_parents(uint32_t V, L0Ranks R, const uint32_t *__restrict__ ckey,
 			     const uint32_t *__restrict__ voff, const uint32_t *__restrict__ loff, const uint32_t *__restrict__ ladj,
 			     const uint32_t *__restrict__ lle,
 			     const uint32_t *__restrict__ ft, const uint32_t *__restrict__ heads,
@@ -597,7 +720,7 @@
 		const uint32_t r = comp_root_side(start_key, voff, g), L = 2 * (voff[g + 1] - voff[g] - 1);
 		t0seg[r >> 1] = make_uint4(NIL, (r & 1u) ? T0_RBIT : 0u, 0u, L ? L - 1 : 0u);
 		const uint32_t h = heads[g];
-		if (h == NIL ? L != 0 : rank_l0(R, trec[h]) != L - 1)
+		if (h == NIL ? L != 0 : rank_l0_of(R, h) != L - 1)
 			atomicExch(err, 1u);
 	}
 	if (g >= V)
@@ -607,15 +730,23 @@
 	uint32_t at_e = NIL, dmin = 0xFFFFFFFFu, dmax = 0u;
 	uint32_t a_l = NIL, a_r = NIL, d_l = 0u, d_r = 0u;
 	for (uint32_t at0 = sb; at0 < se; at0 += 4) {
-		const uint32_t *r32 = reinterpret_cast<const uint32_t *>(trec + at0);
-		const uint4 lw4 = load4_unaligned(lle + at0), r01 = load4_unaligned(r32), r23 = load4_unaligned(r32 + 4);
-		const uint32_t lws[4] = {lw4.x, lw4.y, lw4.z, lw4.w};
-		const uint2 rs[4] = {make_uint2(r01.x, r01.y), make_uint2(r01.z, r01.w), make_uint2(r23.x, r23.y), make_uint2(r23.z, r23.w)};
-		bool tree[4];
+		const uint4 lw4 = load4_unaligned(lle + at0), w4 = load4_unaligned(R.w0 + at0);
+		const uint32_t lws[4] = {lw4.x, lw4.y, lw4.z, lw4.w}, w0s[4] = {w4.x, w4.y, w4.z, w4.w};
+		bool tree[4], esc = false;
+#pragma unroll
+		for (uint32_t q = 0; q < 4; q++) {
+			tree[q] = at0 + q < se && (lws[q] & LLE_TREE);
+			esc |= tree[q] && (w0s[q] & REC_ESC);
+		}
+		uint4 y4 = make_uint4(0u, 0u, 0u, 0u);
+		if (__any(esc))
+			y4 = load4_unaligned(R.w1 + at0);
+		const uint32_t w1s[4] = {y4.x, y4.y, y4.z, y4.w};
+		uint2 rs[4];
 		uint32_t ds[4];
 #pragma unroll
 		for (uint32_t q = 0; q < 4; q++) {
-			tree[q] = at0 + q < se && (lws[q] & LLE_TREE);
+			rs[q] = rec_decode<false>(at0 + q, R.b, w0s[q], w1s[q]);
 			ds[q] = R.ra[l0_at(R, rs[q], tree[q])];
 		}
 		landed(ds[0], ds[1], ds[2], ds[3]);
@@ -1182,7 +1313,7 @@
 }
 
 template <typename OC, typename SC, typename IC>
-__global__ void k_tree_emit(uint32_t nS, const uint2 *__restrict__ erec, L0Ranks R, const uint8_t *__restrict__ merged,
+__global__ void k_tree_emit(uint32_t nS, L0Ranks R, const uint8_t *__restrict__ merged,
 			    const uint2 *__restrict__ dps, const uint32_t *__restrict__ ckey,
 			    const uint32_t *__restrict__ cproc, const uint32_t *__restrict__ voff,
 			    const unsigned long long *__restrict__ start_key, const uint32_t *__restrict__ gid_s,
@@ -1242,16 +1373,23 @@
 	}
 	const uint32_t Nh = 2 * (voff[c + 1] - v0), hd = start_key[c] != ~0ull ? 1u : 0u;
 	const bool fin = *R.fin != 0;
-	const uint4 r01 = load4_unaligned(reinterpret_cast<const uint32_t *>(erec + 3 * g));
-	const uint2 r2 = erec[3 * g + 2];
+	const uint4 w4 = load4_unaligned(R.w0 + 3 * g);
 	const bool two_leaves = !merged[g];
 	const uint4 d4 = *reinterpret_cast<const uint4 *>(dps + 2 * g);
 	const uint32_t o = d4.x == 2 * g + 1 ? 2 * g : 2 * g + 1, e = o ^ 1u;
 	const uint32_t p = (e & 1u) ? d4.z : d4.x;
 	const bool has_p = p != NIL;
 	const uint32_t pp = has_p ? p : e;
-	const uint2 r_p = erec[3 * (pp >> 1)], d_p = dps[pp];
-	const uint2 r0 = make_uint2(r01.x, r01.y), r1 = make_uint2(r01.z, r01.w);
+	const uint32_t xp = 3 * (pp >> 1), wp = R.w0[xp];
+	const uint2 d_p = dps[pp];
+	uint4 y4 = make_uint4(0u, 0u, 0u, 0u);
+	uint32_t yp = 0u;
+	if (__any(fin || ((w4.x | w4.y | (two_leaves ? w4.z : 0u) | (has_p ? wp : 0u)) & REC_ESC))) {
+		y4 = load4_unaligned(R.w1 + 3 * g);
+		yp = R.w1[xp];
+	}
+	const uint2 r0 = rec_decode<true>(3 * g, R.b, w4.x, y4.x, fin), r1 = rec_decode<true>(3 * g + 1, R.b, w4.y, y4.y, fin);
+	const uint2 r2 = rec_decode<true>(3 * g + 2, R.b, w4.z, y4.z, fin), r_p = rec_decode<true>(xp, R.b, wp, yp, fin);
 	const uint32_t i0 = l0_at(R, r0, !fin);
 	uint32_t a0 = R.ra[i0], b0 = R.rb[i0], a1 = R.ra[l0_at(R, r1, !fin)], a2 = R.ra[l0_at(R, r2, !fin && two_leaves)], a_p = R.ra[l0_at(R, r_p, !fin && has_p)];
 	landed(a0, b0, a1, a2, a_p);
@@ -1677,7 +1815,9 @@
 		  bitsA(sparse ? 4u : rank_bucket_bits(n_slots)), bitsE(sparse ? 4u : rank_bucket_bits(n_events)),
 		  rb{tw_.rk_pk, tw_.rk_heads, tw_.rk_nx, tw_.rk_wa, tw_.rk_wb, tw_.rk_tA, tw_.rk_tB, tw_.rk_tC}
 	{
-	}
+		tw.rec_stats[0].valid = tw.rec_stats[1].valid = false;
+	}
+	RankRecStats *rec_stats(int k) { return getenv("POVU_HIP_RANK_STATS") ? &tw.rec_stats[k] : nullptr; }
 	void enqueue_events()
 	{
 		HIP_CHECK(hipMemsetAsync(rb.heads, 0xFF, (size_t)C * 4, s));
@@ -1697,9 +1837,9 @@
 	tw.tour_words_done = false;
 	LAUNCH(k_tour_ends, C, s, C, cs.voff, P.start_key, cs.loff, cs.ladj, cs.lle, P.rb.pk, P.rb.heads);
 	if (P.n_slots)
-		P.tour_r = list_rank_splitters<false>((uint32_t)P.n_slots, P.bitsA, tw.dist, nullptr, C, P.rb, s);
+		P.tour_r = list_rank_splitters<false>((uint32_t)P.n_slots, P.bitsA, tw.dist, nullptr, C, P.rb, s, P.rec_stats(0));
 	HIP_CHECK(hipMemsetAsync(tw.xrec, 0, ((size_t)P.XW + 2) * 16, s));
-	LAUNCH(k_t0_parents, std::max(V, C), s, V, tw.dist, P.tour_r, cs.ckey, cs.voff, cs.loff, cs.ladj, cs.lle, P.v.ft, P.rb.heads,
+	LAUNCH(k_t0_parents, std::max(V, C), s, V, P.tour_r, cs.ckey, cs.voff, cs.loff, cs.ladj, cs.lle, P.v.ft, P.rb.heads,
 	       tw.t0seg, P.v.fstr, tw.xrec, C, P.start_key, P.pw.err + PW_FOREST_SIZE, P.v.multi);
 	P.tm.end(40);
 }
@@ -1805,7 +1945,7 @@
 	P.tm.begin("tree_preorder");
 	if (!P.events_done)
 		P.enqueue_events();
-	P.evr = list_rank_splitters<true, true>(P.n_events, P.bitsE, P.tw.evt, P.pw.err + PW_RANK_OVF, P.C, P.rb, P.s);
+	P.evr = list_rank_splitters<true, true>(P.n_events, P.bitsE, P.tw.evt, P.pw.err + PW_RANK_OVF, P.C, P.rb, P.s, P.rec_stats(1));
 	P.tm.end(40);
 }
 
@@ -1820,7 +1960,7 @@
 		using OC = std::remove_pointer_t<decltype(ordcnt)>;
 		using SC = std::remove_pointer_t<decltype(srccnt)>;
 		using IC = std::remove_pointer_t<decltype(incnt)>;
-		LAUNCH((k_tree_emit<OC, SC, IC>), std::max(P.V, P.C), P.s, P.nS, tw.evt, P.evr, P.v.merged, tw.dps, cs.ckey, tw.cproc, cs.voff, P.start_key, cs.gid_s, sw.t_gid,
+		LAUNCH((k_tree_emit<OC, SC, IC>), std::max(P.V, P.C), P.s, P.nS, P.evr, P.v.merged, tw.dps, cs.ckey, tw.cproc, cs.voff, P.start_key, cs.gid_s, sw.t_gid,
 		       sw.t_flags, sw.t_par, sw.t_size, (sw.hairpins || sw.want_depth) ? sw.t_depth : nullptr, tw.side_tidx, P.C, sw.c_ntree, ordcnt,
 		       pw.hi0, pw.mpre, srccnt, pw.sdl, incnt);
 	};
diff --git a/povu_amd/csrc/hip/tree_kernels.hpp b/povu_amd/csrc/hip/tree_kernels.hpp
--- a/povu_amd/csrc/hip/tree_kernels.hpp
+++ b/povu_amd/csrc/hip/tree_kernels.hpp
@@ -6,6 +6,16 @@
 
 namespace povu_hip
 {
+
+struct RankRecStats {
+	bool valid = false;
+	uint32_t fin = 0;
+	uint32_t bits = 0;
+	uint32_t delta_bits = 0;
+	uint32_t part_bits[2] = {};
+	uint64_t live = 0, esc = 0;
+	uint64_t hist[33 * 33] = {};
+};
 
 struct TreeWs {
 	HostScratch *host;
@@ -34,6 +44,7 @@
 	hipEvent_t walk_fork = nullptr, walk_join = nullptr;
 	Arena *walk_arena = nullptr;
 	bool walk_inline = true;
+	RankRecStats rec_stats[2];
 };
 
 size_t tree_workspace_bytes(size_t V, size_t E, size_t Cmax, int groups = 3, const StageWsOpts &o = StageWsOpts{});
@@ -48,7 +59,8 @@
 			   bool force_big_class_dfs, bool force_sparse_splitters, StageTimer &tm, hipStream_t s);
 
 void debug_list_rank(uint32_t n, const uint32_t *next, const uint8_t *w, const uint32_t *heads, uint32_t nh, int mode,
-		     unsigned bits, uint32_t *ra, uint32_t *rb, hipStream_t s);
+		     unsigned bits, uint32_t *ra, uint32_t *rb, hipStream_t s, RankRecStats *st = nullptr,
+		     std::vector<uint32_t> *plane0 = nullptr);
 
 void edge_id_weights(const CompState &cs, const SeqWs &sw, const TreeWs &tw, uint32_t *w, uint32_t *tail, hipStream_t s);
 
diff --git a/povu_amd/hip.py b/povu_amd/hip.py
--- a/povu_amd/hip.py
+++ b/povu_amd/hip.py
@@ -29,6 +29,11 @@
 
 class _Opts(C.Structure):
     _fields_ = [("rank", C.c_uint32), ("world", C.c_uint32), ("flags", C.c_uint32)]
+
+
+class _RankRecords(C.Structure):
+    _fields_ = [("live", C.c_uint64), ("escaped", C.c_uint64), ("final_ranks", C.c_uint32), ("bucket_bits", C.c_uint32),
+                ("delta_bits", C.c_uint32), ("partial_bits", C.c_uint32 * 2), ("hist", C.c_uint64 * (33 * 33))]
 
 
 class _SubTree(C.Structure):
@@ -342,6 +347,8 @@
                                          C.c_void_p]
     l.povu_hip_debug_append.restype = C.c_int
     l.povu_hip_debug_append.argtypes = [C.c_void_p, C.c_void_p, C.c_size_t, C.c_void_p, C.POINTER(C.c_uint32)]
+    l.povu_hip_debug_rank_escapes.restype = C.c_int
+    l.povu_hip_debug_rank_escapes.argtypes = [C.c_void_p, C.c_int, C.c_void_p, C.c_void_p, C.c_size_t]
     l.povu_hip_debug_list_rank.restype = C.c_int
     l.povu_hip_debug_list_rank.argtypes = [C.c_void_p, C.c_uint32, C.c_void_p, C.c_void_p, C.c_void_p, C.c_uint32,
                                            C.c_int, C.c_uint32, C.c_void_p, C.c_void_p]
@@ -1343,7 +1350,23 @@
                                                 1 if events else 0, bits, ra.ctypes.data, rb.ctypes.data)
         if rc:
             raise RuntimeError(f"debug_list_rank failed ({rc})")
+        self._last_list_rank_n = nxt.size
         return (ra, rb) if events else ra
+
+    def debug_rank_escapes(self, which: str = "list_rank", flags: bool = False):
+        k = {"tour": 0, "events": 1, "list_rank": 2}[which]
+        rec = _RankRecords()
+        esc = np.zeros(self._last_list_rank_n if flags else 0, dtype=np.uint8)
+        rc = self._lib.povu_hip_debug_rank_escapes(self._ctx, k, C.byref(rec), esc.ctypes.data if flags else None, esc.size)
+        if rc:
+            raise RuntimeError(f"debug_rank_escapes failed ({rc})")
+        out = {"live": int(rec.live), "escaped": int(rec.escaped), "final_ranks": bool(rec.final_ranks),
+               "bucket_bits": int(rec.bucket_bits), "delta_bits": int(rec.delta_bits),
+               "partial_bits": (int(rec.partial_bits[0]), int(rec.partial_bits[1])),
+               "hist": np.ctypeslib.as_array(rec.hist).reshape(33, 33).copy()}
+        if flags:
+            out["esc"] = esc
+        return out
 
     def debug_components(self, n_vtx: int):
         comp = np.zeros(n_vtx, dtype=np.uint32)
```

Measured after the change: 3.433 billion, median of 6. 2.0% higher.
